# LeSN-Lab/diff-ViT

Hardware: AMD Instinct MI355X
Metric: images/sec DeiT-S int8 224^2 b=256 (quantized forward) (higher is better)
Workload: dtype int8; 1 GPU; deit_small PoT-PTQ forward, bit_config=[8]*50, 224x224, batch 256 per GPU; global_batch=256, parallelism=dp1, streams_per_gpu=3, collective=none, ranks_seen=1, distinct_devices=1

## Files before the change

### diff-vit_amd/csrc/p2vit_capi.cpp

```cpp
#include <hip/hip_runtime.h>
#include <math.h>
#include <stdarg.h>
#include <stdio.h>
#include <stdlib.h>
#include <string.h>

#include <initializer_list>
#include <memory>
#include <vector>

#include "p2vit_kernels.h"

static thread_local char g_err[512] = "";

static int fail(int code, const char* fmt, ...) {
  va_list ap;
  va_start(ap, fmt);
  vsnprintf(g_err, sizeof g_err, fmt, ap);
  va_end(ap);
  return code;
}
static bool stream_capturing(void* stream) {
  hipStreamCaptureStatus status = hipStreamCaptureStatusNone;
  if (hipStreamIsCapturing((hipStream_t)stream, &status) != hipSuccess) {
    (void)hipGetLastError();
    return false;
  }
  return status == hipStreamCaptureStatusActive;
}
static int refuse_capture(const char* who, const char* why, void* stream) {
  if (!stream_capturing(stream)) return P2V_OK;
  return fail(P2V_E_UNSUPPORTED, "%s: the stream is capturing a HIP graph and this call %s; make it outside the capture", who, why);
}
struct KeepLastError {
  char keep[sizeof g_err];
  KeepLastError() { memcpy(keep, g_err, sizeof keep); }
  ~KeepLastError() { memcpy(g_err, keep, sizeof keep); }
};
static int launch_rc(int rc, const char* what) {
  if (rc == 0) return 0;
  if (rc == -2) return fail(P2V_E_UNSUPPORTED, "%s: s_qkv_sq * inv_s_attn must be a power of two", what);
  if (rc < 0) return fail(P2V_E_UNSUPPORTED, "%s: no kernel instantiated for this shape", what);
  return fail(P2V_E_LAUNCH, "%s: %s", what, hipGetErrorString((hipError_t)rc));
}
static inline int round_up(int v, int m) { return (v + m - 1) / m * m; }
static bool is_pot(float v) {
  int ex;
  return v > 0.f && frexpf(v, &ex) == 0.5f;
}

static int check_lis_consts(const char* who, int x0_int, int b_int, int c_int) {
  if (x0_int >= 0) return fail(P2V_E_ARG, "%s: x0_int must be negative", who);
  if (c_int <= 0 || c_int >= (1 << 24) || b_int < 0 || b_int >= (1 << 23) || x0_int < -(1 << 12))
    return fail(P2V_E_UNSUPPORTED, "%s: log-int-softmax constants out of range (x0 %d, b %d, c %d): softmax input scale below 2^-11?", who, x0_int,
                b_int, c_int);
  return P2V_OK;
}
static int check_requant_scale(const char* who, float inv_s_out) {
  if (!(is_pot(inv_s_out) && inv_s_out >= 0x1p-40f && inv_s_out <= 0x1p40f))
    return fail(P2V_E_UNSUPPORTED, "%s: REQUANT 1/scale %g must be a power of two (it is folded into the column scales)", who, inv_s_out);
  return P2V_OK;
}
static int check_gelu_tab(const char* who, const p2v_gelu_tab& t) {
  if (t.table && (t.cells <= 0 || t.cells > 4096)) return fail(P2V_E_ARG, "%s: GELU table with %d cells", who, t.cells);
  return P2V_OK;
}
static int check_softmax_bits(const char* who, int bits) {
  if (bits != 3 && bits != 4) return fail(P2V_E_UNSUPPORTED, "%s: softmax_bits %d (the log-int-softmax runs at 3 or 4 bits)", who, bits);
  return P2V_OK;
}
static float av_mul_max(int bits) { return bits == 3 ? 0x1p7f : 0x1p15f; }
static int check_attn(const char* who, const p2v_attn& at, int bits = 4) {
  if (const int rb = check_softmax_bits(who, bits)) return rb;
  const int rc = check_lis_consts(who, at.x0_int, at.b_int, at.c_int);
  if (rc != P2V_OK) return rc;
  if (!is_pot(at.s_qkv_sq * at.inv_s_attn)) return fail(P2V_E_UNSUPPORTED, "%s: s_qkv_sq * inv_s_attn must be a power of two", who);
  if (!(at.qk_scale > 0.f) || !(at.av_mul > 0.f)) return fail(P2V_E_ARG, "%s: qk_scale and av_mul must be positive", who);
  if (!is_pot(at.av_mul) || at.av_mul > av_mul_max(bits) || at.av_mul < 0x1p-40f)
    return fail(P2V_E_UNSUPPORTED, "%s: av_mul %g must be a power of two in [2^-40, 2^%d] at softmax_bits %d", who, at.av_mul, bits == 3 ? 7 : 15, bits);
  return P2V_OK;
}

struct p2v_plan {
  p2v_model_desc d;
  int tokens, patches, k_patch, k_patch_pad, n_layers;
  std::vector<p2v_linear> lin[2];
  std::vector<char> lin_set[2];
  float inv_s_input;
  p2v_epilogue embed_epi;
  const int8_t* cls_codes;
  const int8_t* embed_cls_codes = nullptr;
  bool embed_set;
  std::vector<p2v_block> blocks;
  std::vector<char> block_set;
  p2v_ln final_ln;
  float head_inv_s, head_s;
  bool head_set;
  std::vector<float*> ln_pre_buf;
  float* final_pre_buf = nullptr;
  std::vector<char> block_folded;
  std::vector<const float*> resid_tab;
  std::vector<float*> resid_buf;
  int device = -1;
  bool float_norm = false, float_softmax = false, fhead_set = false;
  std::vector<p2v_float_block> fblocks;
  std::vector<char> fblock_set;
  p2v_float_ln final_fln = {};
  std::vector<char> softmax_bits;
  struct GramScale { const float* scale; const uint8_t* shift; double unit; };
  std::vector<GramScale> gram_scales;
  uint8_t* gram_shift_buf = nullptr;
  bool grams_ready = false;
  ~p2v_plan() {
    int prev = -1;
    const bool sw = device >= 0 && hipGetDevice(&prev) == hipSuccess && prev != device && hipSetDevice(device) == hipSuccess;
    for (float* b : ln_pre_buf)
      if (b) (void)hipFree(b);
    for (float* b : resid_buf)
      if (b) (void)hipFree(b);
    if (final_pre_buf) (void)hipFree(final_pre_buf);
    if (gram_shift_buf) (void)hipFree(gram_shift_buf);
    if (sw) (void)hipSetDevice(prev);
  }
};

static void build_resid_tables(p2v_plan* plan, int block);
static int bit_index(int bits) { return bits == 4 ? 0 : (bits == 8 ? 1 : -1); }
template <class Block>
static auto& block_ln(Block& b, int i) { return i < 2 ? b.ln1[i] : b.ln2[(i - 2) >> 1][(i - 2) & 1]; }
static bool ln_constants_present(const p2v_ln& l, bool with_mask = true) {
  return (l.mask || !with_mask) && l.gamma && l.beta && l.inv_out && l.post_mul;
}

extern "C" {

extern int g_ln_generic;
extern int g_ln_rows;
extern int g_attn_waves;
extern int g_ln_gemm;
extern int g_ln_gemm_ver;
extern int g_gemm_tile;
extern int g_resid_pre;
extern int g_attn_stream;
extern int g_attn_packed;
extern int g_ln_pre;
extern int g_gemm_rows;
int g_cls_rows = 1;

enum { ANY_ENV = 1, ANY_API = 2 };
static const struct Switch {
  const char *name, *env;
  int* var;
  int lo, hi, step, any;
  bool takes(int v, int how) const { return (any & how) || (v >= lo && v <= hi && (v - lo) % step == 0); }
  void set(int v) const { *var = (hi == 1 && lo == 0) ? v != 0 : v; }
} kSwitches[] = {
    {"attn_waves", "P2V_ATTN_WAVES", &g_attn_waves, 4, 8, 1, 0},
    {"ln_gemm", "P2V_LN_GEMM", &g_ln_gemm, 0, 1, 1, ANY_ENV | ANY_API},
    {"ln_gemm_version", "P2V_LN_GEMM_V", &g_ln_gemm_ver, 1, 3, 1, 0},
    {"gemm_tile", "P2V_GEMM_TILE", &g_gemm_tile, 0, 256, 128, 0},
    {"attn_stream", "P2V_ATTN_STREAM", &g_attn_stream, 0, 1, 1, ANY_ENV | ANY_API},
    {"attn_packed", "P2V_ATTN_PACKED", &g_attn_packed, 0, 1, 1, 0},
    {"ln_pre", "P2V_LN_PRE", &g_ln_pre, 0, 1, 1, ANY_ENV | ANY_API},
    {"resid_pre", "P2V_RESID_PRE", &g_resid_pre, 0, 1, 1, ANY_ENV | ANY_API},
    {"gemm_rows", "P2V_GEMM_ROWS", &g_gemm_rows, 0, 2, 1, 0},
    {"cls_rows", "P2V_CLS_ROWS", &g_cls_rows, 0, 1, 1, ANY_ENV},
    {"ln_rows", "P2V_LN_ROWS", &g_ln_rows, 1, 64, 1, 0},
    {"ln_generic", "P2V_LN_GENERIC", &g_ln_generic, 0, 1, 1, ANY_API},
};

static void read_env_once() {
  static bool done = false;
  if (done) return;
  done = true;
  for (const Switch& s : kSwitches) {
    const char* e = getenv(s.env);
    if (e && s.takes(atoi(e), ANY_ENV)) s.set(atoi(e));
  }
}
int p2v_abi_version(void) { read_env_once(); return P2V_ABI_VERSION; }

int p2v_resident_tokens(int head_dim) { return p2v_resident_tokens_of(head_dim); }
int p2v_max_tokens(int head_dim) { return p2v_resident_tokens_of(head_dim) ? P2V_MAX_TOKENS_STREAMED : 0; }
int p2v_packed_tokens(int head_dim) { return head_dim == 64 ? P2V_MAX_TOKENS_PACKED : 0; }
int p2v_attention_kernel(int head_dim, int tokens, int tapped) {
  read_env_once();
  return p2v_attention_kernel_of(head_dim, tokens, tapped);
}

int p2v_set_tuning(const char* name, int value) {
  if (!name) return fail(P2V_E_ARG, "p2v_set_tuning: null name");
  read_env_once();
  for (const Switch& s : kSwitches)
    if (!strcmp(name, s.name) && s.takes(value, ANY_API)) {
      s.set(value);
      return P2V_OK;
    }
  return fail(P2V_E_ARG, "p2v_set_tuning: unknown switch or value out of range: %s = %d", name, value);
}
const char* p2v_last_error(void) { return g_err; }

int p2v_plan_create(const p2v_model_desc* desc, p2v_plan** out) {
  if (!desc || !out) return fail(P2V_E_ARG, "p2v_plan_create: null argument");
  read_env_once();
  if (desc->abi_version != P2V_ABI_VERSION) return fail(P2V_E_ARG, "ABI version %d != %d", desc->abi_version, P2V_ABI_VERSION);
  const p2v_model_desc& d = *desc;
  if (d.img_size <= 0 || d.patch_size <= 0 || d.img_size % d.patch_size) return fail(P2V_E_SHAPE, "img_size %% patch_size != 0");
  if (d.patch_size % 4) return fail(P2V_E_UNSUPPORTED, "patch_size must be a multiple of 4");
  if (d.embed_dim % d.num_heads) return fail(P2V_E_SHAPE, "embed_dim %% num_heads != 0");
  const int hd = d.embed_dim / d.num_heads;
  if (hd != 32 && hd != 48 && hd != 64 && hd != 80 && hd != 96 && hd != 128)
    return fail(P2V_E_UNSUPPORTED, "head_dim %d (32, 48, 64, 80, 96 and 128 are instantiated)", hd);
  if (d.embed_dim % 16 || d.mlp_hidden % 16) return fail(P2V_E_UNSUPPORTED, "embed_dim and mlp_hidden must be multiples of 16");
  {
    const int tokens = (d.img_size / d.patch_size) * (d.img_size / d.patch_size) + 1;
    if (tokens > P2V_MAX_TOKENS_STREAMED)
      return fail(P2V_E_UNSUPPORTED, "%d tokens per image: the attention kernels cover up to %d", tokens, P2V_MAX_TOKENS_STREAMED);
  }
  if (d.embed_dim > 2048) return fail(P2V_E_UNSUPPORTED, "embed_dim %d: the LayerNorm kernel covers up to 2048 channels", d.embed_dim);
  p2v_plan* p = new p2v_plan();
  p->d = d;
  p->patches = (d.img_size / d.patch_size) * (d.img_size / d.patch_size);
  p->tokens = p->patches + 1;
  p->k_patch = d.in_chans * d.patch_size * d.patch_size;
  p->k_patch_pad = round_up(p->k_patch, GBK_PAD);
  p->n_layers = 4 * d.depth + 2;
  for (int b = 0; b < 2; ++b) {
    p->lin[b].assign(p->n_layers, p2v_linear{nullptr, nullptr, nullptr, nullptr, 0});
    p->lin_set[b].assign(p->n_layers, 0);
  }
  p->blocks.resize(d.depth);
  p->block_set.assign(d.depth, 0);
  p->ln_pre_buf.assign(d.depth, nullptr);
  p->block_folded.assign(d.depth, 0);
  p->resid_tab.assign((size_t)d.depth * 4, nullptr);
  p->resid_buf.assign(d.depth, nullptr);
  p->embed_set = p->head_set = false;
  p->cls_codes = nullptr;
  p->fblocks.resize(d.depth);
  p->fblock_set.assign(d.depth, 0);
  p->softmax_bits.assign(d.depth, 4);
  *out = p;
  return P2V_OK;
}

void p2v_plan_destroy(p2v_plan* plan) { delete plan; }

int p2v_plan_set_linear(p2v_plan* plan, int layer, int bits, const p2v_linear* lin) {
  if (!plan || !lin) return fail(P2V_E_ARG, "p2v_plan_set_linear: null argument");
  const int bi = bit_index(bits);
  if (bi < 0) return fail(P2V_E_BITS, "bits %d not in {4, 8}", bits);
  if (layer < 0 || layer >= plan->n_layers) return fail(P2V_E_ARG, "layer %d out of range [0,%d)", layer, plan->n_layers);
  if (!lin->w_codes || !lin->colscale || !lin->bias) return fail(P2V_E_ARG, "p2v_plan_set_linear: null device pointer");
  if (lin->packed4 && bits != 4) return fail(P2V_E_BITS, "packed4 weights for a %d-bit layer", bits);
  plan->lin[bi][layer] = *lin;
  plan->lin_set[bi][layer] = 1;
  if (layer >= 1 && layer < plan->n_layers - 1 && ((layer - 1) & 1)) {
    const int block = (layer - 1) / 4;
    if (plan->block_set[block]) build_resid_tables(plan, block);
  }
  return P2V_OK;
}

int p2v_plan_set_embed(p2v_plan* plan, float inv_s_input, const p2v_epilogue* e, const int8_t* cls_row_codes) {
  if (!plan || !e || !cls_row_codes) return fail(P2V_E_ARG, "p2v_plan_set_embed: null argument");
  plan->inv_s_input = inv_s_input;
  plan->embed_epi = *e;
  plan->embed_epi.patches = plan->patches;
  plan->cls_codes = cls_row_codes;
  plan->embed_set = true;
  return P2V_OK;
}

int p2v_plan_set_embed_tap_cls(p2v_plan* plan, const int8_t* cls_embed_codes) {
  if (!plan || !cls_embed_codes) return fail(P2V_E_ARG, "p2v_plan_set_embed_tap_cls: null argument");
  plan->embed_cls_codes = cls_embed_codes;
  return P2V_OK;
}

struct OwnerDevice {
  int prev = -1, own = -1;
  explicit OwnerDevice(const void* ptr) {
    hipPointerAttribute_t pa;
    if (hipGetDevice(&prev) != hipSuccess || hipPointerGetAttributes(&pa, ptr) != hipSuccess) {
      (void)hipGetLastError();
      return;
    }
    if (pa.type != hipMemoryTypeDevice && pa.type != hipMemoryTypeManaged) return;
    own = pa.device;
    if (own != prev && hipSetDevice(own) != hipSuccess) own = -1;
  }
  ~OwnerDevice() { if (own >= 0 && own != prev) (void)hipSetDevice(prev); }
  bool ok() const { return own >= 0; }
};

static size_t resid_tab_floats(int N) { return (size_t)((N + 127) / 128) * 6 * 128; }

static int resid_prefold_impl(const p2v_linear& lin, const p2v_epilogue& ep, int N, float* tab, int* usable, hipStream_t st) {
  *usable = 0;
  unsigned* flags = nullptr;
  hipError_t e = hipMalloc(&flags, 2 * sizeof(unsigned));
  const unsigned init[2] = {1u, 0u};
  unsigned got[2] = {0u, 0u};
  if (e == hipSuccess) e = hipMemcpyAsync(flags, init, sizeof init, hipMemcpyHostToDevice, st);
  int rc = 0;
  if (e == hipSuccess) rc = p2v_launch_resid_prefold(lin, ep, N, tab, flags, st);
  if (e == hipSuccess && rc == 0) e = hipMemcpyAsync(got, flags, sizeof got, hipMemcpyDeviceToHost, st);
  if (e == hipSuccess && rc == 0) e = hipStreamSynchronize(st);
  if (flags) (void)hipFree(flags);
  if (e != hipSuccess) {
    (void)hipGetLastError();
    return fail(P2V_E_LAUNCH, "resid_prefold: %s", hipGetErrorString(e));
  }
  if (rc) return launch_rc(rc, "resid_prefold");
  *usable = got[0] ? 1 : 0;
  return P2V_OK;
}

static void build_resid_tables(p2v_plan* plan, int block) {
  KeepLastError keep;
  for (int j = 0; j < 4; ++j) plan->resid_tab[(size_t)block * 4 + j] = nullptr;
  if (!plan->block_set[block]) return;
  const p2v_block& blk = plan->blocks[block];
  OwnerDevice dev(blk.proj_epi.s_mid);
  if (!dev.ok() || (plan->device >= 0 && plan->device != dev.own)) return;
  const int D = plan->d.embed_dim;
  const size_t per = resid_tab_floats(D);
  if (hipDeviceSynchronize() != hipSuccess) { (void)hipGetLastError(); return; }
  float* buf = plan->resid_buf[block];
  if (!buf && hipMalloc(&buf, 4 * per * sizeof(float)) != hipSuccess) { (void)hipGetLastError(); return; }
  plan->resid_buf[block] = buf;
  plan->device = dev.own;
  for (int which = 0; which < 2; ++which)
    for (int bi = 0; bi < 2; ++bi) {
      const int layer = 1 + 4 * block + (which ? 3 : 1);
      if (!plan->lin_set[bi][layer]) continue;
      int usable = 0;
      float* tab = buf + (size_t)(which * 2 + bi) * per;
      if (resid_prefold_impl(plan->lin[bi][layer], which ? blk.fc2_epi : blk.proj_epi, D, tab, &usable, nullptr) == P2V_OK && usable)
        plan->resid_tab[(size_t)block * 4 + which * 2 + bi] = tab;
    }
}

static hipError_t fold_one_ln(const p2v_ln& l, int C, float* dev, p2v_ln_pre* out) {
  const int Cp = round_up(C, 256);
  std::vector<float> g(C), b(C), io(C), pm(C), host((size_t)2 * Cp, 0.f);
  hipError_t e = hipMemcpy(g.data(), l.gamma, C * sizeof(float), hipMemcpyDeviceToHost);
  if (e == hipSuccess) e = hipMemcpy(b.data(), l.beta, C * sizeof(float), hipMemcpyDeviceToHost);
  if (e == hipSuccess) e = hipMemcpy(io.data(), l.inv_out, C * sizeof(float), hipMemcpyDeviceToHost);
  if (e == hipSuccess) e = hipMemcpy(pm.data(), l.post_mul, C * sizeof(float), hipMemcpyDeviceToHost);
  if (e != hipSuccess) return e;
  float* go = host.data();
  float* bo = go + Cp;
  int pot = 1, pm1 = 1;
  float gmin = 3.0e38f, gmax = 0.f, bmax = 0.f;
  for (int c = 0; c < C; ++c) {
    unsigned ib;
    memcpy(&ib, &io[c], 4);
    const int p2 = (int)((ib & 0x807FFFFFu) == 0u) & (int)((ib >> 23) - 32u <= 190u);
    go[c] = g[c] * io[c];
    bo[c] = b[c] * io[c];
    const float ga = fabsf(go[c]), ba = fabsf(bo[c]);
    const int gok = (int)(g[c] == 0.f) | ((int)(ga >= 1.0e-30f) & (int)(ga <= 1.0e30f));
    const int bok = (int)(b[c] == 0.f) | ((int)(ba >= 1.0e-30f) & (int)(ba <= 1.0e30f));
    pot &= p2 & gok & bok;
    pm1 &= (int)(pm[c] == 1.f);
    gmin = fminf(gmin, ga);
    gmax = fmaxf(gmax, ga);
    bmax = fmaxf(bmax, ba);
  }
  e = hipMemcpy(dev, host.data(), host.size() * sizeof(float), hipMemcpyHostToDevice);
  if (e == hipSuccess) *out = p2v_ln_pre{dev, dev + Cp, gmin, gmax, bmax, pot, pm1};
  return e;
}
static const p2v_ln_pre kNoPre = {nullptr, nullptr, 0.f, 0.f, 0.f, 0, 0};

static bool fold_ln_constants(p2v_plan* plan, int block) {
  const int C = plan->d.embed_dim, Cp = round_up(C, 256);
  p2v_block& blk = plan->blocks[block];
  for (int i = 0; i < 6; ++i) block_ln(blk, i).pre = kNoPre;
  OwnerDevice own(blk.ln1[0].gamma);
  if (!own.ok()) {
    fail(P2V_OK, "p2v_plan_set_block: LayerNorm constants of block %d not folded at plan time (cannot locate the device of gamma)", block);
    return false;
  }
  if (plan->device >= 0 && plan->device != own.own) {
    fail(P2V_OK, "p2v_plan_set_block: block %d lives on device %d, earlier blocks on device %d: not folded at plan time", block, own.own, plan->device);
    return false;
  }
  hipError_t e = hipDeviceSynchronize();
  float* dev = plan->ln_pre_buf[block];
  if (e == hipSuccess && !dev) e = hipMalloc(&dev, (size_t)12 * Cp * sizeof(float));
  p2v_ln_pre pre[6];
  if (e == hipSuccess) {
    plan->ln_pre_buf[block] = dev;
    plan->device = own.own;
    for (int i = 0; i < 6 && e == hipSuccess; ++i) e = fold_one_ln(block_ln(blk, i), C, dev + (size_t)(2 * i) * Cp, &pre[i]);
  }
  if (e != hipSuccess) {
    (void)hipGetLastError();
    fail(P2V_OK, "p2v_plan_set_block: LayerNorm constants of block %d not folded at plan time (%s)", block, hipGetErrorString(e));
    return false;
  }
  for (int i = 0; i < 6; ++i) block_ln(blk, i).pre = pre[i];
  return true;
}

int p2v_plan_set_block(p2v_plan* plan, int block, const p2v_block* blk) {
  if (!plan || !blk) return fail(P2V_E_ARG, "p2v_plan_set_block: null argument");
  if (block < 0 || block >= plan->d.depth) return fail(P2V_E_ARG, "block %d out of range", block);
  int rc = check_attn("p2v_plan_set_block: attn", blk->attn, plan->softmax_bits[block]);
  if (rc == P2V_OK) rc = check_gelu_tab("p2v_plan_set_block: gelu_fc1", blk->gelu_fc1);
  for (int b = 0; b < 2 && rc == P2V_OK; ++b) rc = check_requant_scale("p2v_plan_set_block: inv_s_qkv", blk->inv_s_qkv[b]);
  if (rc == P2V_OK && !(is_pot(blk->inv_s_fc1) && blk->inv_s_fc1 >= 0x1p-40f && blk->inv_s_fc1 <= 0x1p40f))
    rc = fail(P2V_E_UNSUPPORTED, "p2v_plan_set_block: 1/scale of mlp.qact1 %g must be a power of two", blk->inv_s_fc1);
  if (rc == P2V_OK && (!blk->proj_epi.s_mid || !blk->proj_epi.s_res || !blk->proj_epi.s_next || !blk->fc2_epi.s_mid || !blk->fc2_epi.s_res ||
                       !blk->fc2_epi.s_next))
    rc = fail(P2V_E_ARG, "p2v_plan_set_block: RESID epilogues need s_mid/s_res/s_next");
  for (int i = 0; i < 6 && rc == P2V_OK; ++i)
    if (!ln_constants_present(block_ln(*blk, i))) rc = fail(P2V_E_ARG, "p2v_plan_set_block: LayerNorm constants missing");
  if (rc != P2V_OK) return rc;
  plan->blocks[block] = *blk;
  plan->block_set[block] = 1;
  g_err[0] = 0;
  plan->block_folded[block] = fold_ln_constants(plan, block) ? 1 : 0;
  build_resid_tables(plan, block);
  return P2V_OK;
}

int p2v_plan_block_prefolded(const p2v_plan* plan, int block) {
  if (!plan || block < 0 || block >= plan->d.depth) return fail(P2V_E_ARG, "p2v_plan_block_prefolded: bad argument");
  return plan->block_folded[block] ? 1 : 0;
}

int p2v_plan_resid_prefolded(const p2v_plan* plan, int block) {
  if (!plan || block < 0 || block >= plan->d.depth) return fail(P2V_E_ARG, "p2v_plan_resid_prefolded: bad argument");
  int m = 0;
  for (int j = 0; j < 4; ++j) m |= plan->resid_tab[(size_t)block * 4 + j] ? 1 << j : 0;
  return m;
}

int p2v_plan_set_head(p2v_plan* plan, const p2v_ln* final_ln, float inv_s_out, float s_out) {
  if (!plan || !final_ln) return fail(P2V_E_ARG, "p2v_plan_set_head: null argument");
  if (!ln_constants_present(*final_ln))
    return fail(P2V_E_ARG, "p2v_plan_set_head: LayerNorm constants missing");
  if (!(inv_s_out > 0.f) || !(s_out > 0.f)) return fail(P2V_E_ARG, "p2v_plan_set_head: act_out scale must be positive");
  plan->final_ln = *final_ln;
  plan->final_ln.pre = kNoPre;
  {
    OwnerDevice own(final_ln->gamma);
    const int C = plan->d.embed_dim;
    if (own.ok() && (plan->device < 0 || plan->device == own.own) && hipDeviceSynchronize() == hipSuccess) {
      if (!plan->final_pre_buf && hipMalloc(&plan->final_pre_buf, (size_t)2 * round_up(C, 256) * sizeof(float)) != hipSuccess) plan->final_pre_buf = nullptr;
      p2v_ln_pre pre;
      if (plan->final_pre_buf && fold_one_ln(*final_ln, C, plan->final_pre_buf, &pre) == hipSuccess) {
        plan->final_ln.pre = pre;
        plan->device = own.own;
      }
    }
    (void)hipGetLastError();
  }
  plan->head_inv_s = inv_s_out;
  plan->head_s = s_out;
  plan->head_set = true;
  return P2V_OK;
}

struct WsLayout {
  size_t patches, x, ln, qkv, att, hid, cls, total;
};
static WsLayout ws_layout(const p2v_plan* p, int batch) {
// ... 1807 lines not shown
```

### diff-vit_amd/csrc/p2vit_ln.hip

```cpp
#include "p2vit_ln_row.h"
#include "p2vit_launch.h"


#ifndef LN_BATCH
#define LN_BATCH 2
#endif
#ifndef LN_LDSC
#define LN_LDSC true
#endif
template <int NCH, int LANES, bool PRE, bool TAP = false>
__global__ __launch_bounds__(256) void k_int_layernorm(LnArgs a) {
  __shared__ __attribute__((aligned(16))) float sG[NCH * LANES * 4], sB[NCH * LANES * 4], sP[NCH * LANES * 4];
  __shared__ __attribute__((aligned(16))) int sM[NCH * LANES * 4];
  const int tid = threadIdx.x, l32 = tid & (LANES - 1), hw = tid / LANES;
  LnLane<NCH, LN_LDSC> L;
  const int LN_ROWS = a.rows_per_half;
  const long long row0 = ((long long)blockIdx.x * (256 / LANES) + hw) * LN_ROWS;
  const long long last_row = a.rows - 1;
  constexpr int R = LN_BATCH;
  int colofs[NCH];
#pragma unroll
  for (int i = 0; i < NCH; ++i) colofs[i] = (l32 + LANES * i) * 4 < a.C ? (l32 + LANES * i) * 4 : 0;
  unsigned wnext[R][NCH];
#pragma unroll
  for (int u = 0; u < R; ++u)
#pragma unroll
    for (int i = 0; i < NCH; ++i)
      wnext[u][i] = *reinterpret_cast<const unsigned*>(a.x + (row0 + u < a.rows ? row0 + u : last_row) * a.row_stride + colofs[i]);
  if constexpr (PRE) {
#pragma unroll
    for (int i = 0; i < NCH; ++i) {
      const int c = (l32 + LANES * i) * 4;
      L.on[i] = c < a.C;
      L.gm[i] = *reinterpret_cast<const float4*>(a.pre.gm + c);
      L.bt[i] = *reinterpret_cast<const float4*>(a.pre.bt + c);
    }
    for (int t4 = tid; t4 < NCH * LANES; t4 += 256) {
      const int c = t4 * 4;
      float4 pmv = make_float4(0.f, 0.f, 0.f, 0.f), mk = pmv;
      if (c < a.C) {
        pmv = *reinterpret_cast<const float4*>(a.ln.post_mul + c);
        mk = *reinterpret_cast<const float4*>(a.ln.mask + c);
      }
      *reinterpret_cast<float4*>(sP + c) = pmv;
      *reinterpret_cast<float4*>(sM + c) = ln_scale_mask(mk);
    }
    __syncthreads();
#pragma unroll
    for (int i = 0; i < NCH; ++i) {
      const int c = (l32 + LANES * i) * 4;
      if constexpr (sizeof(L.pm) == sizeof(float4) * NCH) {
        L.pm[i] = *reinterpret_cast<const float4*>(sP + c);
        L.mkf[i] = *reinterpret_cast<const float4*>(sM + c);
      }
    }
    L.sPl = sP + l32 * 4;
    L.sMl = reinterpret_cast<const float*>(sM) + l32 * 4;
    L.cstride = LANES * 4;
    L.gmin = a.pre.gmin;
    L.gmax = a.pre.gmax;
    L.bmax = a.pre.bmax;
    L.pot = a.pre.pot != 0 && a.force_generic == 0;
    L.pm_one = a.pre.pm_one != 0;
  } else {
    ln_prepare<NCH, LANES>(a.ln, a.C, a.force_generic != 0, sG, sB, sP, sM, tid, 256, L);
  }
#pragma unroll
  for (int u = 0; u < R; ++u)
#pragma unroll
    for (int i = 0; i < NCH; ++i) asm volatile("" : "+v"(wnext[u][i]));
#pragma unroll 1
  for (int rr = 0; rr < LN_ROWS; rr += R) {
    const long long row = row0 + rr;
    if (row >= a.rows) break;
    unsigned wcur[R][NCH];
#pragma unroll
    for (int u = 0; u < R; ++u)
#pragma unroll
      for (int i = 0; i < NCH; ++i) wcur[u][i] = L.on[i] ? wnext[u][i] : 0u;
#pragma unroll
    for (int u = 0; u < R; ++u) {
      const long long nrow = row + R + u < a.rows ? row + R + u : last_row;
#pragma unroll
      for (int i = 0; i < NCH; ++i) wnext[u][i] = *reinterpret_cast<const unsigned*>(a.x + nrow * a.row_stride + colofs[i]);
    }
    asm volatile("" ::: "memory");
    unsigned outw[R][NCH];
    if constexpr (TAP) {
      float* taps[R];
#pragma unroll
      for (int u = 0; u < R; ++u) taps[u] = (rr + u < LN_ROWS && row + u < a.rows) ? a.tap_out + (row + u) * (long long)a.C : nullptr;
      if constexpr (R == 1) ln_row<NCH, LANES, decltype(L), true>(wcur[0], L, a.ln, a.C, l32, outw[0], taps[0]);
      else ln_rows<NCH, LANES, R, decltype(L), true>(wcur, L, a.ln, a.C, l32, outw, taps);
    } else {
    if constexpr (R == 1) ln_row<NCH, LANES>(wcur[0], L, a.ln, a.C, l32, outw[0]);
    else ln_rows<NCH, LANES, R>(wcur, L, a.ln, a.C, l32, outw);
    }
#pragma unroll
    for (int u = 0; u < R; ++u)
#pragma unroll
      for (int i = 0; i < NCH; ++i) asm volatile("" : "+v"(wnext[u][i]));
#pragma unroll
    for (int u = 0; u < R; ++u) {
      if (rr + u >= LN_ROWS || row + u >= a.rows) continue;
      int8_t* dst = a.out + (row + u) * a.out_stride;
#pragma unroll
      for (int i = 0; i < NCH; ++i)
        if (L.on[i]) *reinterpret_cast<unsigned*>(dst + (l32 + LANES * i) * 4) = outw[u][i];
    }
  }
}

#define LG_BM 64
template <bool W4> struct LgW { typedef uint4 raw; };
template <> struct LgW<true> { typedef uint2 raw; };
__device__ __forceinline__ v4i lg_wfrag(uint4 w) { return __builtin_bit_cast(v4i, w); }
__device__ __forceinline__ v4i lg_wfrag(uint2 w) { return unpack_w4(w.x, w.y); }
struct LnGemmLds {
  int panel, consts, fold, table, total;
};
__host__ __device__ inline LnGemmLds ln_gemm_lds(int K, int N, int nch, int table_cells) {
  LnGemmLds o;
  const int kt = (K + GBK - 1) / GBK, tiles_n = (N + GBN - 1) / GBN;
  o.panel = 0;
  o.consts = o.panel + kt * LG_BM * GBK;
  o.fold = o.panel;
  o.table = o.consts + tiles_n * GBN * 2 * (int)sizeof(float);
  o.total = o.table + table_cells * 8;
  return o;
}

#ifdef P2V_DIAG
#define LG_STAMP(slot)                                                                                              \
  do {                                                                                                              \
    if (g.stamps && threadIdx.x == 0 && (slot) < 62) g.stamps[(long long)blockIdx.x * 64 + (slot)] = __builtin_readcyclecounter(); \
  } while (0)
#else
#define LG_STAMP(slot) do { } while (0)
#endif
template <int EPI, int KT, bool W4>
__global__ __launch_bounds__(256, 2) void k_ln_gemm(LnArgs a, GemmArgs g) {
  typedef typename LgW<W4>::raw wraw;
  constexpr int NCH = (KT + 1) / 2;
  constexpr int NI = 2 * KT;
  extern __shared__ __attribute__((aligned(1024))) unsigned char lg_smem[];
  LG_STAMP(0);
  const int C = a.C;
  const int cells = EPI == P2V_EPI_GELU_TAB ? g.ep.gelu.cells : 0;
  const LnGemmLds lay = ln_gemm_lds(C, g.N, NCH, cells);
  int8_t* panel = reinterpret_cast<int8_t*>(lg_smem + lay.panel);
  float* consts = reinterpret_cast<float*>(lg_smem + lay.consts);
  const unsigned char* gtab = lg_smem + lay.table;
  const int tid = threadIdx.x, lane = tid & 63;
  const int wave = __builtin_amdgcn_readfirstlane(tid >> 6);
  const int h = lane >> 5, l31 = lane & 31;
  const int m0 = blockIdx.x * LG_BM;
  const int tiles_n = g.tiles_n;

  const wraw* wsrc = reinterpret_cast<const wraw*>(g.W) + (long long)wave * NI * 64 + lane;
  wraw wf[NI];
#pragma unroll
  for (int i = 0; i < NI; ++i) wf[i] = wsrc[i * 64];

  constexpr int RPH = LG_BM / 8;
  static_assert(RPH % 2 == 0, "rows are processed in pairs");
  const int hw = tid >> 5;
  auto load_row = [&](int r, unsigned (&w)[NCH]) {
    long long row = (long long)m0 + hw * RPH + r;
    row = row < a.rows ? row : a.rows - 1;
#pragma unroll
    for (int i = 0; i < NCH; ++i) {
      const int c = (l31 + 32 * i) * 4;
      w[i] = *reinterpret_cast<const unsigned*>(a.x + row * a.row_stride + (c < C ? c : 0));
    }
  };
  unsigned win[2][NCH];
  load_row(0, win[0]);
  load_row(1, win[1]);
  {
    const float fold = EPI == P2V_EPI_REQUANT ? g.ep.inv_s_out : (EPI == P2V_EPI_GELU_TAB ? g.ep.gelu.k : 1.0f);
    const float cfold = fold * (W4 ? 0.0625f : 1.0f);
    for (int n4 = tid; n4 < tiles_n * (GBN / 4); n4 += 256) {
      const int j_ = n4 >> 5, c_ = (n4 & 31) * 4;
      const float4 cv = *reinterpret_cast<const float4*>(g.colscale + n4 * 4);
      const float4 bv = *reinterpret_cast<const float4*>(g.bias + n4 * 4);
      *reinterpret_cast<float4*>(consts + j_ * 2 * GBN + c_) = make_float4(cv.x * cfold, cv.y * cfold, cv.z * cfold, cv.w * cfold);
      *reinterpret_cast<float4*>(consts + j_ * 2 * GBN + GBN + c_) = make_float4(bv.x * fold, bv.y * fold, bv.z * fold, bv.w * fold);
    }
    if (EPI == P2V_EPI_GELU_TAB)
      for (int i = tid; i < cells; i += 256)
        reinterpret_cast<uint2*>(lg_smem + lay.table)[i] = reinterpret_cast<const uint2*>(g.ep.gelu.table)[i];
  }
  LG_STAMP(1);
  {
    float* sG = reinterpret_cast<float*>(lg_smem + lay.fold);
    float* sB = sG + NCH * 128;
    float* sP = sB + NCH * 128;
    int* sM = reinterpret_cast<int*>(sP + NCH * 128);
    LnLane<NCH> L;
    ln_prepare<NCH, 32>(a.ln, C, a.force_generic != 0, sG, sB, sP, sM, tid, 256, L);
    __syncthreads();
#pragma unroll 1
    for (int r = 0; r < RPH; r += 2) {
      unsigned wnext[2][NCH];
      if (r + 2 < RPH) {
        load_row(r + 2, wnext[0]);
        load_row(r + 3, wnext[1]);
      }
      unsigned wcur[2][NCH], outw2[2][NCH];
#pragma unroll
      for (int u = 0; u < 2; ++u)
#pragma unroll
        for (int i = 0; i < NCH; ++i) wcur[u][i] = L.on[i] ? win[u][i] : 0u;
      ln_rows<NCH, 32, 2>(wcur, L, a.ln, C, l31, outw2);
#pragma unroll
      for (int u = 0; u < 2; ++u) {
        const int lrow = hw * RPH + r + u;
        const unsigned (&outw)[NCH] = outw2[u];
        const long long row = (long long)m0 + lrow;
#pragma unroll
        for (int i = 0; i < NCH; ++i) {
          const int c = (l31 + 32 * i) * 4;
          if (c < KT * GBK)
            *reinterpret_cast<unsigned*>(panel + (c >> 6) * (LG_BM * GBK) + lrow * GBK + ((((c & 63) >> 4) ^ ((lrow >> 2) & 3)) << 4) + (c & 15)) =
                L.on[i] ? outw[i] : 0u;
          if (a.out && L.on[i] && row < a.rows) *reinterpret_cast<unsigned*>(a.out + row * a.out_stride + c) = outw[i];
        }
      }
      if (r + 2 < RPH) {
#pragma unroll
        for (int i = 0; i < NCH; ++i) {
          win[0][i] = wnext[0][i];
          win[1][i] = wnext[1][i];
        }
      }
    }
  }
  LG_STAMP(2);
  __syncthreads();
  LG_STAMP(3);

  const int8_t* pXa = panel + lds_off64(l31, h);
  const int8_t* pXb = panel + lds_off64(32 + l31, h);
  const int xks = (lds_off64(l31, 2 + h) - lds_off64(l31, h));
  v16i acc[2];
#pragma unroll
  for (int b = 0; b < 2; ++b)
#pragma unroll
    for (int r = 0; r < 16; ++r) acc[b][r] = 0;

  for (int j = 0; j < tiles_n; ++j) {
    const bool more = j + 1 < tiles_n;
    const wraw* wnext = wsrc + (long long)(more ? j + 1 : j) * 4 * NI * 64;
#pragma unroll
    for (int i = 0; i < NI; ++i) {
      const int off = (i >> 1) * (LG_BM * GBK) + (i & 1) * xks;
      const v4i xa = *reinterpret_cast<const v4i*>(pXa + off);
      const v4i xb = *reinterpret_cast<const v4i*>(pXb + off);
      const v4i wfi = lg_wfrag(wf[i]);
      acc[0] = __builtin_amdgcn_mfma_i32_32x32x32_i8(wfi, xa, acc[0], 0, 0, 0);
      acc[1] = __builtin_amdgcn_mfma_i32_32x32x32_i8(wfi, xb, acc[1], 0, 0, 0);
      wf[i] = wnext[i * 64];
    }
    LG_STAMP(4 + 2 * j);
    const EpiLds* e = reinterpret_cast<const EpiLds*>(consts + j * 2 * GBN);
    {
      const uint4 nores[2] = {make_uint4(0, 0, 0, 0), make_uint4(0, 0, 0, 0)};
      gemm_epilogue_tile2<EPI>(acc, m0 + l31, j * GBN + 32 * wave, 32 * wave, h, g, e, nores, gtab);
#pragma unroll
      for (int mi = 0; mi < 2; ++mi)
#pragma unroll
        for (int r = 0; r < 16; ++r) acc[mi][r] = 0;
    }
    LG_STAMP(5 + 2 * j);
  }
}

template <int NI>
__host__ __device__ constexpr int lg2_mfma_at(int hp) {
  for (int q = 0; q < 2 * NI; ++q)
    if ((q * 12) / NI == hp) return q;
  return -1;
}

#ifndef LG2_LN_ROWS
#define LG2_LN_ROWS 2
#endif
template <int EPI, int KT, int NG, bool W4>
__global__ __launch_bounds__(256 * NG, 2) void k_ln_gemm2(LnArgs a, GemmArgs g) {
  typedef typename LgW<W4>::raw wraw;
  constexpr int NT = 256 * NG;
  static_assert(EPI == P2V_EPI_REQUANT || EPI == P2V_EPI_GELU_TAB, "pipelined epilogues");
  constexpr int NCH = (KT + 1) / 2;
  constexpr int NI = 2 * KT;
  extern __shared__ __attribute__((aligned(1024))) unsigned char lg_smem[];
  LG_STAMP(0);
  const int C = a.C;
  const int cells = EPI == P2V_EPI_GELU_TAB ? g.ep.gelu.cells : 0;
  const LnGemmLds lay = ln_gemm_lds(C, g.N, NCH, cells);
  int8_t* panel = reinterpret_cast<int8_t*>(lg_smem + lay.panel);
  float* consts = reinterpret_cast<float*>(lg_smem + lay.consts);
  const unsigned char* gtab = lg_smem + lay.table;
  const int tid = threadIdx.x, lane = tid & 63;
  const int wave = __builtin_amdgcn_readfirstlane(tid >> 6);
  const int grp = NG == 1 ? 0 : (wave >> 2), cw = wave & 3;
  const int h = lane >> 5, l31 = lane & 31;
  const int m0 = blockIdx.x * LG_BM;
  const int tiles_n = g.tiles_n;
  const int n_g = (tiles_n - grp + NG - 1) / NG;

  const wraw* wsrc = reinterpret_cast<const wraw*>(g.W) + (long long)cw * NI * 64 + lane;
  auto wtile = [&](int it) {
    int j = grp + NG * it;
    j = j < tiles_n ? j : tiles_n - 1;
    return wsrc + (long long)j * 4 * NI * 64;
  };
  constexpr int NI_EARLY = KT >= 6 ? NI - 1 : NI;
  wraw wf[NI];
  {
    const wraw* w0 = wtile(0);
#pragma unroll
    for (int i = 0; i < NI_EARLY; ++i) wf[i] = w0[i * 64];
  }

  constexpr int RPH = LG_BM / (8 * NG);
  static_assert(RPH % 2 == 0, "rows are processed in pairs");
  const int hw = tid >> 5;
  const int8_t* xblk = a.x + (long long)m0 * a.row_stride;
  const int rstride = (int)a.row_stride;
  const int last_lr = (int)(a.rows - 1 - m0);
  auto load_row = [&](int r, unsigned (&w)[NCH]) {
    int lr = hw * RPH + r;
    lr = lr < last_lr ? lr : last_lr;
    const int8_t* rp = xblk + lr * rstride;
#pragma unroll
    for (int i = 0; i < NCH; ++i) {
      const int c = (l31 + 32 * i) * 4;
      w[i] = *reinterpret_cast<const unsigned*>(rp + (c < C ? c : 0));
    }
  };
  constexpr int LR = LG2_LN_ROWS < RPH ? LG2_LN_ROWS : RPH;
  static_assert(RPH % LR == 0, "rows are processed in batches");
  unsigned win[LR][NCH];
#pragma unroll
  for (int u = 0; u < LR; ++u) load_row(u, win[u]);
  {
    const float fold = EPI == P2V_EPI_REQUANT ? g.ep.inv_s_out : (EPI == P2V_EPI_GELU_TAB ? g.ep.gelu.k : 1.0f);
    const float cfold = fold * (W4 ? 0.0625f : 1.0f);
    for (int n4 = tid; n4 < tiles_n * (GBN / 4); n4 += NT) {
      const int j_ = n4 >> 5, c_ = (n4 & 31) * 4;
      const float4 cv = *reinterpret_cast<const float4*>(g.colscale + n4 * 4);
      const float4 bv = *reinterpret_cast<const float4*>(g.bias + n4 * 4);
      *reinterpret_cast<float4*>(consts + j_ * 2 * GBN + c_) = make_float4(cv.x * cfold, cv.y * cfold, cv.z * cfold, cv.w * cfold);
      *reinterpret_cast<float4*>(consts + j_ * 2 * GBN + GBN + c_) = make_float4(bv.x * fold, bv.y * fold, bv.z * fold, bv.w * fold);
    }
    if (EPI == P2V_EPI_GELU_TAB)
      for (int i = tid; i < cells; i += NT)
        reinterpret_cast<uint2*>(lg_smem + lay.table)[i] = reinterpret_cast<const uint2*>(g.ep.gelu.table)[i];
  }
  LG_STAMP(1);
  {
    float* sG = reinterpret_cast<float*>(lg_smem + lay.fold);
    float* sB = sG + NCH * 128;
    float* sP = sB + NCH * 128;
    int* sM = reinterpret_cast<int*>(sP + NCH * 128);
    LnLane<NCH> L;
    if (a.pre.gm) {
#pragma unroll
      for (int i = 0; i < NCH; ++i) {
        const int c = (l31 + 32 * i) * 4;
        L.on[i] = c < C;
        L.gm[i] = *reinterpret_cast<const float4*>(a.pre.gm + c);
        L.bt[i] = *reinterpret_cast<const float4*>(a.pre.bt + c);
        L.pm[i] = L.on[i] ? *reinterpret_cast<const float4*>(a.ln.post_mul + c) : make_float4(0.f, 0.f, 0.f, 0.f);
        L.mkf[i] = L.on[i] ? ln_scale_mask(*reinterpret_cast<const float4*>(a.ln.mask + c)) : make_float4(0.f, 0.f, 0.f, 0.f);
      }
      L.gmin = a.pre.gmin;
      L.gmax = a.pre.gmax;
      L.bmax = a.pre.bmax;
      L.pot = a.pre.pot != 0 && a.force_generic == 0;
      L.pm_one = a.pre.pm_one != 0;
    } else {
      ln_prepare<NCH, 32>(a.ln, C, a.force_generic != 0, sG, sB, sP, sM, tid, NT, L);
      __syncthreads();
    }
#pragma unroll 1
    for (int r = 0; r < RPH; r += LR) {
      unsigned wnext[LR][NCH];
      if (r + LR < RPH) {
#pragma unroll
        for (int u = 0; u < LR; ++u) load_row(r + LR + u, wnext[u]);
      }
      unsigned wcur[LR][NCH], outw2[LR][NCH];
#pragma unroll
      for (int u = 0; u < LR; ++u)
#pragma unroll
        for (int i = 0; i < NCH; ++i) wcur[u][i] = L.on[i] ? win[u][i] : 0u;
      ln_rows<NCH, 32, LR>(wcur, L, a.ln, C, l31, outw2);
#pragma unroll
      for (int u = 0; u < LR; ++u) {
        const int lrow = hw * RPH + r + u;
        const unsigned (&outw)[NCH] = outw2[u];
        const long long row = (long long)m0 + lrow;
#pragma unroll
        for (int i = 0; i < NCH; ++i) {
          const int c = (l31 + 32 * i) * 4;
          if (c < KT * GBK)
            *reinterpret_cast<unsigned*>(panel + (c >> 6) * (LG_BM * GBK) + lrow * GBK + ((((c & 63) >> 4) ^ ((lrow >> 2) & 3)) << 4) + (c & 15)) =
                L.on[i] ? outw[i] : 0u;
          if (a.out && L.on[i] && row < a.rows) *reinterpret_cast<unsigned*>(a.out + row * a.out_stride + c) = outw[i];
        }
      }
      if (r + LR < RPH) {
#pragma unroll
        for (int u = 0; u < LR; ++u)
#pragma unroll
          for (int i = 0; i < NCH; ++i) win[u][i] = wnext[u][i];
      }
    }
  }
  LG_STAMP(2);
  if constexpr (NI_EARLY < NI) wf[NI - 1] = wtile(0)[(NI - 1) * 64];
  __syncthreads();
  LG_STAMP(3);
  if (n_g <= 0) return;

  const int8_t* pXa = panel + lds_off64(l31, h);
  const int8_t* pXb = panel + lds_off64(32 + l31, h);
  const int xks = (lds_off64(l31, 2 + h) - lds_off64(l31, h));
#define LG2_XOFF(i) ((((i) >> 1) * (LG_BM * GBK)) + (((i) & 1) ? xks : 0))
  v16i acc[2], accn[2];
#pragma unroll
  for (int b = 0; b < 2; ++b)
#pragma unroll
    for (int r = 0; r < 16; ++r) acc[b][r] = 0;
  {
    const wraw* wn = wtile(1);
#pragma unroll
    for (int i = 0; i < NI; ++i) {
      const v4i xa = *reinterpret_cast<const v4i*>(pXa + LG2_XOFF(i));
      const v4i xb = *reinterpret_cast<const v4i*>(pXb + LG2_XOFF(i));
      const v4i wfi = lg_wfrag(wf[i]);
      acc[0] = __builtin_amdgcn_mfma_i32_32x32x32_i8(wfi, xa, acc[0], 0, 0, 0);
      acc[1] = __builtin_amdgcn_mfma_i32_32x32x32_i8(wfi, xb, acc[1], 0, 0, 0);
      wf[i] = wn[i * 64];
    }
  }
  LG_STAMP(4);
  v4i XA[2], XB[2];
  XA[0] = *reinterpret_cast<const v4i*>(pXa + LG2_XOFF(0));
  XB[0] = *reinterpret_cast<const v4i*>(pXb + LG2_XOFF(0));
  XA[1] = XA[0];
  XB[1] = XB[0];
  const int goff = (int)g.ep.gelu.off;
  const float glo = (float)-goff, ghi = (float)(cells - 1 - goff) + 0.5f;
  const unsigned char* gtabz = gtab + goff * 8;

  v4i wcur = {0, 0, 0, 0};
  auto tile_body = [&](auto MFc, auto LDc, auto COPYc, int j, const wraw* wnn, v16i (&acc)[2], v16i (&accn)[2]) {
    constexpr bool MF = decltype(MFc)::value, LD = decltype(LDc)::value, COPY = decltype(COPYc)::value;
    const float* cst = consts + j * 2 * GBN + 32 * cw + 4 * h;
    const int n_tile = j * GBN + 32 * cw;
    unsigned d[2][4];
    float4 cs = *reinterpret_cast<const float4*>(cst), bs = *reinterpret_cast<const float4*>(cst + GBN);
#define LG2_MFMA(HP)                                                                                                     \
    do {                                                                                                                 \
      constexpr int q_ = lg2_mfma_at<NI>(HP);                                                                            \
      if constexpr (MF && q_ >= 0) {                                                                                     \
        constexpr int i_ = q_ >> 1, nx_ = (i_ + 1) % NI;                                                                 \
        if constexpr ((q_ & 1) == 0) {                                                                                   \
          XA[nx_ & 1] = *reinterpret_cast<const v4i*>(pXa + LG2_XOFF(nx_));                                              \
          wcur = lg_wfrag(wf[i_]);                                                                                       \
          if constexpr (i_ == 0) accn[0] = __builtin_amdgcn_mfma_i32_32x32x32_i8(wcur, XA[i_ & 1], (v16i){0,0,0,0,0,0,0,0,0,0,0,0,0,0,0,0}, 0, 0, 0); \
          else accn[0] = __builtin_amdgcn_mfma_i32_32x32x32_i8(wcur, XA[i_ & 1], accn[0], 0, 0, 0);                      \
        } else {                                                                                                         \
          XB[nx_ & 1] = *reinterpret_cast<const v4i*>(pXb + LG2_XOFF(nx_));                                              \
          if constexpr (i_ == 0) accn[1] = __builtin_amdgcn_mfma_i32_32x32x32_i8(wcur, XB[i_ & 1], (v16i){0,0,0,0,0,0,0,0,0,0,0,0,0,0,0,0}, 0, 0, 0); \
          else accn[1] = __builtin_amdgcn_mfma_i32_32x32x32_i8(wcur, XB[i_ & 1], accn[1], 0, 0, 0);                      \
          if constexpr (LD) wf[i_] = wnn[i_ * 64];                                                                       \
        }                                                                                                                \
      }                                                                                                                  \
    } while (0)
#define LG2_FENCE() __builtin_amdgcn_sched_barrier(0)
    auto group = [&](auto GQc) {
      constexpr int gq = decltype(GQc)::value;
      const float4 csc = cs, bsc = bs;
      if (gq < 3) {
        cs = *reinterpret_cast<const float4*>(cst + 8 * (gq + 1));
        bs = *reinterpret_cast<const float4*>(cst + GBN + 8 * (gq + 1));
      }
      float y0[4], y1[4];
      LG2_MFMA(6 * gq + 0);
      y0[0] = __builtin_fmaf((float)acc[0][4 * gq + 0], csc.x, bsc.x);
      y0[1] = __builtin_fmaf((float)acc[0][4 * gq + 1], csc.y, bsc.y);
      y0[2] = __builtin_fmaf((float)acc[0][4 * gq + 2], csc.z, bsc.z);
      y0[3] = __builtin_fmaf((float)acc[0][4 * gq + 3], csc.w, bsc.w);
      LG2_FENCE();
      LG2_MFMA(6 * gq + 1);
      y1[0] = __builtin_fmaf((float)acc[1][4 * gq + 0], csc.x, bsc.x);
      y1[1] = __builtin_fmaf((float)acc[1][4 * gq + 1], csc.y, bsc.y);
      y1[2] = __builtin_fmaf((float)acc[1][4 * gq + 2], csc.z, bsc.z);
      y1[3] = __builtin_fmaf((float)acc[1][4 * gq + 3], csc.w, bsc.w);
      LG2_FENCE();
      if constexpr (EPI == P2V_EPI_GELU_TAB) {
        uint2 e0[4], e1[4];
        LG2_MFMA(6 * gq + 2);
#pragma unroll
        for (int i = 0; i < 4; ++i) e0[i] = *reinterpret_cast<const uint2*>(gtabz + gelu_tab_offset(y0[i], glo, ghi));
        LG2_FENCE();
        LG2_MFMA(6 * gq + 3);
#pragma unroll
        for (int i = 0; i < 4; ++i) e1[i] = *reinterpret_cast<const uint2*>(gtabz + gelu_tab_offset(y1[i], glo, ghi));
        LG2_FENCE();
        LG2_MFMA(6 * gq + 4);
        d[0][gq] = 0;
        P2V_GELU_SEL(0, "UNUSED_PAD", d[0][gq], y0[0], e0[0]);
        P2V_GELU_SEL(1, "UNUSED_PRESERVE", d[0][gq], y0[1], e0[1]);
        P2V_GELU_SEL(2, "UNUSED_PRESERVE", d[0][gq], y0[2], e0[2]);
        P2V_GELU_SEL(3, "UNUSED_PRESERVE", d[0][gq], y0[3], e0[3]);
        LG2_FENCE();
        LG2_MFMA(6 * gq + 5);
        d[1][gq] = 0;
        P2V_GELU_SEL(0, "UNUSED_PAD", d[1][gq], y1[0], e1[0]);
        P2V_GELU_SEL(1, "UNUSED_PRESERVE", d[1][gq], y1[1], e1[1]);
        P2V_GELU_SEL(2, "UNUSED_PRESERVE", d[1][gq], y1[2], e1[2]);
        P2V_GELU_SEL(3, "UNUSED_PRESERVE", d[1][gq], y1[3], e1[3]);
        LG2_FENCE();
      } else {
        float r0[4], r1[4];
        LG2_MFMA(6 * gq + 2);
#pragma unroll
        for (int i = 0; i < 4; ++i) r0[i] = pre_pack(y0[i]);
        LG2_FENCE();
        LG2_MFMA(6 * gq + 3);
#pragma unroll
        for (int i = 0; i < 4; ++i) r1[i] = pre_pack(y1[i]);
        LG2_FENCE();
        LG2_MFMA(6 * gq + 4);
        d[0][gq] = pack4_pre(r0[0], r0[1], r0[2], r0[3]);
        LG2_FENCE();
        LG2_MFMA(6 * gq + 5);
        d[1][gq] = pack4_pre(r1[0], r1[1], r1[2], r1[3]);
        LG2_FENCE();
      }
    };
    group(std::integral_constant<int, 0>{});
    group(std::integral_constant<int, 1>{});
    group(std::integral_constant<int, 2>{});
    group(std::integral_constant<int, 3>{});
#undef LG2_MFMA
#undef LG2_FENCE
#pragma unroll
    for (int b = 0; b < 2; ++b) {
      const uint4 o = halves_to_row16(d[b][0], d[b][1], d[b][2], d[b][3]);
      const int m = m0 + 32 * b + l31;
      if (m < g.M && n_tile + 16 * h < g.N)
        *reinterpret_cast<uint4*>(reinterpret_cast<int8_t*>(g.out) + (long long)m * g.ldo + n_tile + 16 * h) = o;
    }
    if constexpr (MF && COPY) {
      acc[0] = accn[0];
      acc[1] = accn[1];
    }
  };
  using T_ = std::integral_constant<bool, true>;
  using F_ = std::integral_constant<bool, false>;
  int it = 0;
  for (; it + 3 < n_g; it += 2) {
    tile_body(T_{}, T_{}, F_{}, grp + NG * it, wtile(it + 2), acc, accn);
    LG_STAMP(5 + it);
    tile_body(T_{}, T_{}, F_{}, grp + NG * (it + 1), wtile(it + 3), accn, acc);
    LG_STAMP(6 + it);
  }
  if (it + 2 < n_g) {
    tile_body(T_{}, T_{}, T_{}, grp + NG * it, wtile(it + 2), acc, accn);
    LG_STAMP(5 + it);
    ++it;
  }
  if (it + 1 < n_g) {
    tile_body(T_{}, F_{}, T_{}, grp + NG * it, wsrc, acc, accn);
    LG_STAMP(5 + it);
    ++it;
  }
  tile_body(F_{}, F_{}, T_{}, grp + NG * it, wsrc, acc, accn);
  LG_STAMP(5 + it);
#undef LG2_XOFF
}


#ifdef P2V_DIAG
extern unsigned long long* g_gemm_stamps;
#endif
int g_ln_pre = 1;
int g_ln_generic = 0;
int g_ln_gemm = 1;
bool p2v_ln_gemm_supported(int epi, int C, int N, int table_cells) {
  if (!g_ln_gemm || (epi != P2V_EPI_REQUANT && epi != P2V_EPI_GELU)) return false;
  if (C % 4 || C > 384 || N % 16) return false;
  return ln_gemm_lds(C, N, ((C + GBK - 1) / GBK + 1) / 2, table_cells).total <= 80 * 1024;
}
template <int EPI, int KT, int VER, bool W4>
static int launch_ln_gemm_t(const LnArgs& a, const GemmArgs& g, int cells, hipStream_t st) {
  constexpr auto kernel = [] {
    if constexpr (VER == 1) return &k_ln_gemm<EPI, KT, W4>;
    else return &k_ln_gemm2<EPI, KT, VER - 1, W4>;
  }();
  const int smem = ln_gemm_lds(a.C, g.N, (KT + 1) / 2, cells).total;
  static P2vLdsGrant grant = {};
  const hipError_t e = grant.ensure(reinterpret_cast<const void*>(kernel), smem);
  if (e != hipSuccess) return (int)e;
  const dim3 grid((unsigned)((g.M + LG_BM - 1) / LG_BM));
  hipLaunchKernelGGL(kernel, grid, dim3(VER == 3 ? 512 : 256), (unsigned)smem, st, a, g);
  CHECK_LAUNCH();
  return 0;
}
typedef int (*LnGemmLauncher)(const LnArgs&, const GemmArgs&, int, hipStream_t);
constexpr int kLnGemmEpi[3] = {P2V_EPI_REQUANT, P2V_EPI_GELU_TAB, P2V_EPI_GELU};
constexpr int ln_gemm_index(int e, int ver, int kt, bool w4) { return (((3 - ver) * 3 + p2v_slot(kLnGemmEpi, e)) * 6 + kt - 1) * 2 + (w4 ? 0 : 1); }
struct LnGemmAt {
  template <int I> static constexpr LnGemmLauncher at() {
    constexpr int E = kLnGemmEpi[I / 12 % 3], VER = 3 - I / 36;
    static_assert(ln_gemm_index(E, VER, I / 2 % 6 + 1, !(I & 1)) == I, "decoded as the launcher encodes");
    if constexpr (E != P2V_EPI_GELU || VER == 1) return launch_ln_gemm_t<E, I / 2 % 6 + 1, VER, !(I & 1)>;
    else return nullptr;
  }
};
static const auto ln_gemm_table = p2v_table<LnGemmLauncher, LnGemmAt, 108>();

int g_ln_gemm_ver = 2;
int p2v_launch_ln_gemm(int epi, const LnArgs& a_, const GemmArgs& g0, hipStream_t st) {
  const int cells = (epi == P2V_EPI_GELU && g0.ep.gelu.table) ? g0.ep.gelu.cells : 0;
  if (!p2v_ln_gemm_supported(epi, a_.C, g0.N, cells)) return -3;
  if (a_.row_stride < 0 || a_.row_stride > (1 << 24)) return -3;
  LnArgs a = a_;
  a.force_generic = g_ln_generic;
  if (!g_ln_pre) a.pre.gm = nullptr;
  GemmArgs g = g0;
  g.tiles_n = (g.N + GBN - 1) / GBN;
#ifdef P2V_DIAG
  g.stamps = g_gemm_stamps;
#endif
  const int kt = (a.C + GBK - 1) / GBK;
  const int e = epi == P2V_EPI_REQUANT ? P2V_EPI_REQUANT : (cells ? P2V_EPI_GELU_TAB : P2V_EPI_GELU);
  const int ver = ((g_ln_gemm_ver == 3 || g_ln_gemm_ver == 2) && !g.ep.tap_out && e != P2V_EPI_GELU) ? g_ln_gemm_ver : 1;
  const LnGemmLauncher launch = ln_gemm_table[ln_gemm_index(e, ver, kt >= 1 && kt <= 5 ? kt : 6, g.w4 != 0)];
  return launch ? launch(a, g, cells, st) : -3;
}

typedef void (*LnKernel)(LnArgs);
constexpr int ln_index(bool tap, bool half, int nch, bool pre) { return (((tap ? 0 : 2) + (half ? 1 : 0)) * 9 + nch) * 2 + (pre ? 0 : 1); }
struct LnAt {
  template <int I> static constexpr LnKernel at() {
    constexpr bool HALF = (I / 18 & 1) != 0;
    constexpr int NCH = I / 2 % 9;
    static_assert(ln_index(I < 36, HALF, NCH, !(I & 1)) == I, "decoded as the launcher encodes");
    if constexpr (HALF ? (NCH >= 1 && NCH <= 3) : (NCH >= 2 && NCH <= 8)) return k_int_layernorm<NCH, HALF ? 32 : 64, !(I & 1), (I < 36)>;
    else return nullptr;
  }
};
static const auto ln_table = p2v_table<LnKernel, LnAt, 72>();

int g_ln_rows = 4;
int p2v_launch_layernorm(const LnArgs& a_, hipStream_t st) {
  LnArgs a = a_;
  a.force_generic = g_ln_generic;
  if (!g_ln_pre) a.pre.gm = nullptr;
  if (a.C > 2048) return a.tap_out ? -1 : p2v_launch_layernorm_xwide(a, st);
  a.rows_per_half = g_ln_rows;
  const int LN_ROWS = g_ln_rows;
  const bool wide = a.C > 384;
  const int nch = wide ? (a.C + 255) / 256 : (a.C + 127) / 128;
  const int rows_per_block = (wide ? 4 : 8) * LN_ROWS;
  dim3 grid((unsigned)((a.rows + rows_per_block - 1) / rows_per_block)), block(256);
  const LnKernel kernel = (nch >= 0 && nch <= 8) ? ln_table[ln_index(a.tap_out != nullptr, !wide, nch, a.pre.gm != nullptr)] : nullptr;
  if (!kernel) return -1;
  hipLaunchKernelGGL(kernel, grid, block, 0, st, a);
  CHECK_LAUNCH();
  return 0;
}
```

### diff-vit_amd/csrc/p2vit_ln_row.h

```cpp
#pragma once
#include "p2vit_epilogue.h"

__device__ __forceinline__ int half_wave_sum(int v) {
  v += __builtin_amdgcn_update_dpp(0, v, 0xB1, 0xF, 0xF, false);
  v += __builtin_amdgcn_update_dpp(0, v, 0x4E, 0xF, 0xF, false);
  v += __builtin_amdgcn_update_dpp(0, v, 0x141, 0xF, 0xF, false);
  v += __builtin_amdgcn_update_dpp(0, v, 0x140, 0xF, 0xF, false);
  v += __builtin_amdgcn_ds_swizzle(v, 0x401F);
  return v;
}

__device__ __forceinline__ float ln_elem_generic_o(float xq, float g, float bta, float io, float rs, float mos, float os) {
  const float A = os > 0.f ? (rs * g) / os : (rs * g) * io;
  const float absA = fabsf(A);
  int N = 134 - (int)(__float_as_uint(absA) >> 23);
  N = N < 0 ? 0 : (N > 31 ? 31 : N);
  const float M = fminf(floorf(ldexpf(absA, N)), 255.f);
  const float sM = copysignf(M, A);
  const float tb = bta - mos * g;
  const float Bv = rintf(ldexpf(os > 0.f ? tb / os : tb * io, N));
  return rintf(ldexpf(sM * xq + Bv, -N));
}
__device__ __forceinline__ float ln_elem_generic(float xq, float g, float bta, float io, float pm, float rs, float mos, float os) {
  const float o = ln_elem_generic_o(xq, g, bta, io, rs, mos, os);
  return rintf(o * pm);
}

#define LN_XS 0x1p-16f
#define LN_XS_INV 65536.f
__device__ __forceinline__ float4 ln_scale_mask(float4 m) { return make_float4(m.x * LN_XS, m.y * LN_XS, m.z * LN_XS, m.w * LN_XS); }
template <int NCH, bool LDSC = false>
struct LnLane {
  bool on[NCH];
  float4 gm[NCH], bt[NCH];
  float4 pm[LDSC ? 1 : NCH];
  float4 mkf[LDSC ? 1 : NCH];
  const float* sPl;
  const float* sMl;
  int cstride;
  float gmin, gmax;
  float bmax;
  bool pot;
  bool pm_one;
  __device__ __forceinline__ float4 post4(int i) const { return LDSC ? *reinterpret_cast<const float4*>(sPl + i * cstride) : pm[LDSC ? 0 : i]; }
  __device__ __forceinline__ float4 mask4(int i) const { return LDSC ? *reinterpret_cast<const float4*>(sMl + i * cstride) : mkf[LDSC ? 0 : i]; }
};

template <int NCH, int LANES, class LL>
__device__ __forceinline__ void ln_prepare(const p2v_ln& ln, int C, bool force_generic, float* sG, float* sB, float* sP, int* sM,
                                           int tid, int nthreads, LL& L) {
  const int l32 = tid & (LANES - 1);
  int potf = force_generic ? 0 : 1, pm1 = 1;
  for (int t4 = tid; t4 < NCH * LANES; t4 += nthreads) {
    const int c = t4 * 4;
    float4 g = make_float4(0.f, 0.f, 0.f, 0.f), b = g, io = make_float4(1.f, 1.f, 1.f, 1.f), pmv = g, mk = g;
    if (c < C) {
      g = *reinterpret_cast<const float4*>(ln.gamma + c);
      b = *reinterpret_cast<const float4*>(ln.beta + c);
      io = *reinterpret_cast<const float4*>(ln.inv_out + c);
      pmv = *reinterpret_cast<const float4*>(ln.post_mul + c);
      mk = *reinterpret_cast<const float4*>(ln.mask + c);
    }
    const float g4[4] = {g.x, g.y, g.z, g.w}, b4[4] = {b.x, b.y, b.z, b.w}, i4[4] = {io.x, io.y, io.z, io.w};
    if (c < C) pm1 &= (int)(pmv.x == 1.f) & (int)(pmv.y == 1.f) & (int)(pmv.z == 1.f) & (int)(pmv.w == 1.f);
    float go[4], bo[4];
#pragma unroll
    for (int j = 0; j < 4; ++j) {
      const unsigned ib = __float_as_uint(i4[j]);
      const int p2 = (int)((ib & 0x807FFFFFu) == 0u) & (int)((ib >> 23) - 32u <= 190u);
      go[j] = g4[j] * i4[j];
      bo[j] = b4[j] * i4[j];
      const float ga = fabsf(go[j]), ba = fabsf(bo[j]);
      const int gok = (int)(g4[j] == 0.f) | ((int)(ga >= 1.0e-30f) & (int)(ga <= 1.0e30f));
      const int bok = (int)(b4[j] == 0.f) | ((int)(ba >= 1.0e-30f) & (int)(ba <= 1.0e30f));
      potf &= p2 & gok & bok;
    }
    *reinterpret_cast<float4*>(sG + c) = make_float4(go[0], go[1], go[2], go[3]);
    *reinterpret_cast<float4*>(sB + c) = make_float4(bo[0], bo[1], bo[2], bo[3]);
    *reinterpret_cast<float4*>(sP + c) = pmv;
    *reinterpret_cast<float4*>(sM + c) = ln_scale_mask(mk);
  }
  L.pot = __syncthreads_and(potf) != 0;
  L.pm_one = __syncthreads_and(pm1) != 0;
  float gmin = 3.0e38f, gmax = 0.f, bmax = 0.f;
#pragma unroll
  for (int i = 0; i < NCH; ++i) {
    const int c = (l32 + LANES * i) * 4;
    L.on[i] = c < C;
    const float4 gv = *reinterpret_cast<const float4*>(sG + c);
    L.gm[i] = gv;
    L.bt[i] = *reinterpret_cast<const float4*>(sB + c);
    if (L.on[i]) bmax = fmaxf(bmax, fmaxf(fmaxf(fabsf(L.bt[i].x), fabsf(L.bt[i].y)), fmaxf(fabsf(L.bt[i].z), fabsf(L.bt[i].w))));
    if constexpr (sizeof(L.pm) == sizeof(float4) * NCH) {
      L.pm[i] = *reinterpret_cast<const float4*>(sP + c);
      L.mkf[i] = *reinterpret_cast<const float4*>(sM + c);
    }
    const float lo = fminf(fminf(fabsf(gv.x), fabsf(gv.y)), fminf(fabsf(gv.z), fabsf(gv.w)));
    const float hi = fmaxf(fmaxf(fabsf(gv.x), fabsf(gv.y)), fmaxf(fabsf(gv.z), fabsf(gv.w)));
    gmin = fminf(gmin, L.on[i] ? lo : 3.0e38f);
    gmax = fmaxf(gmax, L.on[i] ? hi : 0.f);
  }
  L.sPl = sP + l32 * 4;
  L.sMl = reinterpret_cast<const float*>(sM) + l32 * 4;
  L.cstride = LANES * 4;
  {
    int lo = (int)__float_as_uint(gmin), hi = (int)__float_as_uint(gmax), bh = (int)__float_as_uint(bmax);
#define LN_MM(ctrl) lo = min(lo, __builtin_amdgcn_update_dpp(lo, lo, ctrl, 0xF, 0xF, false)); hi = max(hi, __builtin_amdgcn_update_dpp(hi, hi, ctrl, 0xF, 0xF, false)); \
                    bh = max(bh, __builtin_amdgcn_update_dpp(bh, bh, ctrl, 0xF, 0xF, false));
    LN_MM(0xB1) LN_MM(0x4E) LN_MM(0x141) LN_MM(0x140)
#undef LN_MM
    lo = min(lo, __builtin_amdgcn_ds_swizzle(lo, 0x401F));
    hi = max(hi, __builtin_amdgcn_ds_swizzle(hi, 0x401F));
    bh = max(bh, __builtin_amdgcn_ds_swizzle(bh, 0x401F));
    if (LANES >= 64) {
      lo = min(lo, __shfl_xor(lo, 32));
      hi = max(hi, __shfl_xor(hi, 32));
      bh = max(bh, __shfl_xor(bh, 32));
    }
    L.gmin = __uint_as_float((unsigned)lo);
    L.gmax = __uint_as_float((unsigned)hi);
    L.bmax = __uint_as_float((unsigned)bh);
  }
}

template <int NCH, class LL>
__device__ __forceinline__ void ln_sums(const unsigned (&wcur)[NCH], const LL& L, float (&xq)[NCH][4], int& S1, unsigned& S2) {
  S2 = 0;
  float S1p = 0.f, S2p = 0.f;
#pragma unroll
  for (int i = 0; i < NCH; ++i) {
    const unsigned w = wcur[i];
    const float4 mk_ = L.mask4(i);
    const float m4[4] = {mk_.x, mk_.y, mk_.z, mk_.w};
#pragma unroll
    for (int j = 0; j < 4; ++j) xq[i][j] = (float)sx8(w, j) * m4[j];
    S1p += (xq[i][0] + xq[i][1]) + (xq[i][2] + xq[i][3]);
    S2p += __builtin_fmaf(xq[i][1], xq[i][1], xq[i][0] * xq[i][0]) + __builtin_fmaf(xq[i][3], xq[i][3], xq[i][2] * xq[i][2]);
    if ((i & 3) == 3 || i == NCH - 1) {
      S2 += (unsigned)(S2p * (LN_XS_INV * LN_XS_INV));
      S2p = 0.f;
    }
  }
  S1 = (int)(S1p * LN_XS_INV);
}
template <int LANES>
__device__ __forceinline__ void ln_reduce(int& S1, unsigned& S2) {
  S1 = half_wave_sum(S1);
  S2 = (unsigned)half_wave_sum((int)S2);
  if (LANES == 64) {
    S1 += __shfl_xor(S1, 32);
    S2 += (unsigned)__shfl_xor((int)S2, 32);
  }
}
template <int NCH, class LL>
__device__ __forceinline__ void ln_scalars(int S1, unsigned S2, const LL& L, const p2v_ln& ln, int C, float& rs, float& mos, bool& fast) {
  const float s1 = ln.s1;
  const float Cf = (float)C;
  const float s1oC = s1 / Cf;
  const float S1f = (float)S1, S2f = (float)S2;
  const float mean = (S1f / Cf) * s1;
  const float stdv = s1oC * sqrtf(Cf * S2f - S1f * S1f);
  rs = s1 / stdv;
  mos = mean / stdv;
  const float amin = rs * L.gmin;
  const float tlim = __uint_as_float((((__float_as_uint(amin) >> 23) & 255u) + 15u) << 23);
  fast = L.pot && amin >= 0x1p-24f && rs * L.gmax < 256.f && (L.bmax + fabsf(mos) * L.gmax) * 1.01f < tlim;
}
__device__ __forceinline__ void ln_tap_store(float* tap, int c, const p2v_ln& ln, const float (&o)[4]) {
  float4 os;
  if (ln.out_scale) {
    os = *reinterpret_cast<const float4*>(ln.out_scale + c);
  } else {
    const float4 io = *reinterpret_cast<const float4*>(ln.inv_out + c);
    os = make_float4(1.0f / io.x, 1.0f / io.y, 1.0f / io.z, 1.0f / io.w);
  }
  *reinterpret_cast<float4*>(tap + c) = make_float4(o[0] * os.x, o[1] * os.y, o[2] * os.z, o[3] * os.w);
}

template <int NCH, int LANES, class LL, bool TAP = false>
__device__ __forceinline__ void ln_apply(const float (&xq)[NCH][4], const LL& L, const p2v_ln& ln, int l32, float rs, float mos, bool fast,
                                         unsigned (&outw)[NCH], float* tap = nullptr) {
  if (fast) {
    const float rs2 = rs * LN_XS_INV;
    auto chain = [&](auto PM1c) {
      constexpr bool PM1 = decltype(PM1c)::value;
#pragma unroll
      for (int i = 0; i < NCH; ++i) {
        const float g4[4] = {L.gm[i].x, L.gm[i].y, L.gm[i].z, L.gm[i].w}, b4[4] = {L.bt[i].x, L.bt[i].y, L.bt[i].z, L.bt[i].w};
        float p4[4] = {1.f, 1.f, 1.f, 1.f};
        if constexpr (!PM1) {
          const float4 pm_ = L.post4(i);
          p4[0] = pm_.x; p4[1] = pm_.y; p4[2] = pm_.z; p4[3] = pm_.w;
        }
        float q[4];
        float ot[TAP ? 4 : 1];
#pragma unroll
        for (int j = 0; j < 4; j += 2) {
          v2f T2, Bq2;
#pragma unroll
          for (int e = 0; e < 2; ++e) {
            const float A2 = rs2 * g4[j + e];
            const float t = b4[j + e] - mos * g4[j + e];
            const unsigned Ab = __float_as_uint(A2);
            T2[e] = __uint_as_float(Ab & 0xFFFF0000u);
            unsigned Cmb;
            asm("v_and_or_b32 %0, %1, %2, %3" : "=v"(Cmb) : "v"(Ab), "s"(0x7F800000u), "v"(0x00400000u));
            const float Cm = __uint_as_float(Cmb);
            Bq2[e] = (t + Cm) - Cm;
          }
          const v2f x2 = {xq[i][j], xq[i][j + 1]};
          const v2f o2 = __builtin_elementwise_fma(T2, x2, Bq2);
          if (PM1) {
            q[j] = o2[0];
            q[j + 1] = o2[1];
          } else {
            q[j] = rintf(o2[0]) * p4[j];
            q[j + 1] = rintf(o2[1]) * p4[j + 1];
          }
          if constexpr (TAP) {
            ot[j] = rintf(o2[0]);
            ot[j + 1] = rintf(o2[1]);
          }
        }
        outw[i] = pack4_rne_sat(q[0], q[1], q[2], q[3]);
        if constexpr (TAP)
          if (tap && L.on[i]) ln_tap_store(tap, (l32 + LANES * i) * 4, ln, ot);
      }
    };
    if (L.pm_one) chain(std::integral_constant<bool, true>{});
    else chain(std::integral_constant<bool, false>{});
  } else {
#pragma unroll
    for (int i = 0; i < NCH; ++i) {
      const int cc = L.on[i] ? (l32 + LANES * i) * 4 : 0;
      const float4 gv = *reinterpret_cast<const float4*>(ln.gamma + cc), bv = *reinterpret_cast<const float4*>(ln.beta + cc);
      const float4 iv = *reinterpret_cast<const float4*>(ln.inv_out + cc), pv = *reinterpret_cast<const float4*>(ln.post_mul + cc);
      const float g4[4] = {gv.x, gv.y, gv.z, gv.w}, b4[4] = {bv.x, bv.y, bv.z, bv.w};
      const float i4[4] = {iv.x, iv.y, iv.z, iv.w}, p4[4] = {pv.x, pv.y, pv.z, pv.w};
      float4 ov = make_float4(0.f, 0.f, 0.f, 0.f);
      if (ln.out_scale) ov = *reinterpret_cast<const float4*>(ln.out_scale + cc);
      const float o4[4] = {ov.x, ov.y, ov.z, ov.w};
      float q[4];
      if constexpr (TAP) {
        float ot[4];
#pragma unroll
        for (int j = 0; j < 4; ++j) {
          ot[j] = ln_elem_generic_o(xq[i][j] * LN_XS_INV, g4[j], b4[j], i4[j], rs, mos, o4[j]);
          q[j] = rintf(ot[j] * p4[j]);
        }
        if (tap && L.on[i]) ln_tap_store(tap, cc, ln, ot);
      } else {
#pragma unroll
        for (int j = 0; j < 4; ++j) q[j] = ln_elem_generic(xq[i][j] * LN_XS_INV, g4[j], b4[j], i4[j], p4[j], rs, mos, o4[j]);
      }
      outw[i] = pack4_sat(q[0], q[1], q[2], q[3]);
    }
  }
}

template <int NCH, int LANES, class LL, bool TAP = false>
__device__ __forceinline__ void ln_row(const unsigned (&wcur)[NCH], const LL& L, const p2v_ln& ln, int C, int l32, unsigned (&outw)[NCH],
                                       float* tap = nullptr) {
  float xq[NCH][4], rs, mos;
  int S1;
  unsigned S2;
  bool fast;
  ln_sums<NCH>(wcur, L, xq, S1, S2);
  ln_reduce<LANES>(S1, S2);
  ln_scalars<NCH>(S1, S2, L, ln, C, rs, mos, fast);
  ln_apply<NCH, LANES, LL, TAP>(xq, L, ln, l32, rs, mos, fast, outw, tap);
}

template <int NCH, int LANES, int R, class LL, bool TAP = false>
__device__ __forceinline__ void ln_rows(const unsigned (&wcur)[R][NCH], const LL& L, const p2v_ln& ln, int C, int l32, unsigned (&outw)[R][NCH],
                                        float* const* taps = nullptr) {
  static_assert((R & (R - 1)) == 0 && R <= 8, "rows per batch");
  float xq[R][NCH][4];
  int S1k = 0;
  unsigned S2k = 0;
  const int mine = l32 & (R - 1);
#pragma unroll
  for (int r = 0; r < R; ++r) {
    int S1;
    unsigned S2;
    ln_sums<NCH>(wcur[r], L, xq[r], S1, S2);
    ln_reduce<LANES>(S1, S2);
    S1k = mine == r ? S1 : S1k;
    S2k = mine == r ? S2 : S2k;
  }
  float rs, mos;
  bool fast;
  ln_scalars<NCH>(S1k, S2k, L, ln, C, rs, mos, fast);
  const int fasti = fast ? 1 : 0;
#pragma unroll
  for (int r = 0; r < R; ++r) {
    const float rs_r = __shfl(rs, r, LANES), mos_r = __shfl(mos, r, LANES);
    const bool fast_r = __shfl(fasti, r, LANES) != 0;
    ln_apply<NCH, LANES, LL, TAP>(xq[r], L, ln, l32, rs_r, mos_r, fast_r, outw[r], TAP ? taps[r] : nullptr);
  }
}
```

Before: 107,700 images/sec.

## Add lean LN-GEMM kernel variants with paired DPP reductions behind a switch

Moves the fused layernorm+GEMM kernels into a shared header and adds lean kernel forms (VER 4/5) built in a separate translation unit, chosen through a new ln_gemm_lean switch. It also adds a half-wave reduction that sums two row statistics at once with DPP halving, cutting cross-lane shuffle instructions in the LN prologue. The goal is a shorter LN stage inside the fused kernel. The new code is large, and part of it is not visible here, so dispatch and correctness are hard to confirm.

```diff
diff --git a/diff-vit_amd/csrc/p2vit_capi.cpp b/diff-vit_amd/csrc/p2vit_capi.cpp
--- a/diff-vit_amd/csrc/p2vit_capi.cpp
+++ b/diff-vit_amd/csrc/p2vit_capi.cpp
@@ -139,6 +139,7 @@
 extern int g_attn_waves;
 extern int g_ln_gemm;
 extern int g_ln_gemm_ver;
+extern int g_ln_gemm_lean;
 extern int g_gemm_tile;
 extern int g_resid_pre;
 extern int g_attn_stream;
@@ -167,6 +168,7 @@
     {"cls_rows", "P2V_CLS_ROWS", &g_cls_rows, 0, 1, 1, ANY_ENV},
     {"ln_rows", "P2V_LN_ROWS", &g_ln_rows, 1, 64, 1, 0},
     {"ln_generic", "P2V_LN_GENERIC", &g_ln_generic, 0, 1, 1, ANY_API},
+    {"ln_gemm_lean", "P2V_LN_GEMM_LEAN", &g_ln_gemm_lean, 0, 1, 1, ANY_ENV | ANY_API},
 };
 
 static void read_env_once() {
diff --git a/diff-vit_amd/csrc/p2vit_ln.hip b/diff-vit_amd/csrc/p2vit_ln.hip
--- a/diff-vit_amd/csrc/p2vit_ln.hip
+++ b/diff-vit_amd/csrc/p2vit_ln.hip
@@ -111,480 +111,8 @@
   }
 }
 
-#define LG_BM 64
-template <bool W4> struct LgW { typedef uint4 raw; };
-template <> struct LgW<true> { typedef uint2 raw; };
-__device__ __forceinline__ v4i lg_wfrag(uint4 w) { return __builtin_bit_cast(v4i, w); }
-__device__ __forceinline__ v4i lg_wfrag(uint2 w) { return unpack_w4(w.x, w.y); }
-struct LnGemmLds {
-  int panel, consts, fold, table, total;
-};
-__host__ __device__ inline LnGemmLds ln_gemm_lds(int K, int N, int nch, int table_cells) {
-  LnGemmLds o;
-  const int kt = (K + GBK - 1) / GBK, tiles_n = (N + GBN - 1) / GBN;
-  o.panel = 0;
-  o.consts = o.panel + kt * LG_BM * GBK;
-  o.fold = o.panel;
-  o.table = o.consts + tiles_n * GBN * 2 * (int)sizeof(float);
-  o.total = o.table + table_cells * 8;
-  return o;
-}
+#include "p2vit_ln_gemm.h"
 
-#ifdef P2V_DIAG
-#define LG_STAMP(slot)                                                                                              \
-  do {                                                                                                              \
-    if (g.stamps && threadIdx.x == 0 && (slot) < 62) g.stamps[(long long)blockIdx.x * 64 + (slot)] = __builtin_readcyclecounter(); \
-  } while (0)
-#else
-#define LG_STAMP(slot) do { } while (0)
-#endif
-template <int EPI, int KT, bool W4>
-__global__ __launch_bounds__(256, 2) void k_ln_gemm(LnArgs a, GemmArgs g) {
-  typedef typename LgW<W4>::raw wraw;
-  constexpr int NCH = (KT + 1) / 2;
-  constexpr int NI = 2 * KT;
-  extern __shared__ __attribute__((aligned(1024))) unsigned char lg_smem[];
-  LG_STAMP(0);
-  const int C = a.C;
-  const int cells = EPI == P2V_EPI_GELU_TAB ? g.ep.gelu.cells : 0;
-  const LnGemmLds lay = ln_gemm_lds(C, g.N, NCH, cells);
-  int8_t* panel = reinterpret_cast<int8_t*>(lg_smem + lay.panel);
-  float* consts = reinterpret_cast<float*>(lg_smem + lay.consts);
-  const unsigned char* gtab = lg_smem + lay.table;
-  const int tid = threadIdx.x, lane = tid & 63;
-  const int wave = __builtin_amdgcn_readfirstlane(tid >> 6);
-  const int h = lane >> 5, l31 = lane & 31;
-  const int m0 = blockIdx.x * LG_BM;
-  const int tiles_n = g.tiles_n;
-
-  const wraw* wsrc = reinterpret_cast<const wraw*>(g.W) + (long long)wave * NI * 64 + lane;
-  wraw wf[NI];
-#pragma unroll
-  for (int i = 0; i < NI; ++i) wf[i] = wsrc[i * 64];
-
-  constexpr int RPH = LG_BM / 8;
-  static_assert(RPH % 2 == 0, "rows are processed in pairs");
-  const int hw = tid >> 5;
-  auto load_row = [&](int r, unsigned (&w)[NCH]) {
-    long long row = (long long)m0 + hw * RPH + r;
-    row = row < a.rows ? row : a.rows - 1;
-#pragma unroll
-    for (int i = 0; i < NCH; ++i) {
-      const int c = (l31 + 32 * i) * 4;
-      w[i] = *reinterpret_cast<const unsigned*>(a.x + row * a.row_stride + (c < C ? c : 0));
-    }
-  };
-  unsigned win[2][NCH];
-  load_row(0, win[0]);
-  load_row(1, win[1]);
-  {
-    const float fold = EPI == P2V_EPI_REQUANT ? g.ep.inv_s_out : (EPI == P2V_EPI_GELU_TAB ? g.ep.gelu.k : 1.0f);
-    const float cfold = fold * (W4 ? 0.0625f : 1.0f);
-    for (int n4 = tid; n4 < tiles_n * (GBN / 4); n4 += 256) {
-      const int j_ = n4 >> 5, c_ = (n4 & 31) * 4;
-      const float4 cv = *reinterpret_cast<const float4*>(g.colscale + n4 * 4);
-      const float4 bv = *reinterpret_cast<const float4*>(g.bias + n4 * 4);
-      *reinterpret_cast<float4*>(consts + j_ * 2 * GBN + c_) = make_float4(cv.x * cfold, cv.y * cfold, cv.z * cfold, cv.w * cfold);
-      *reinterpret_cast<float4*>(consts + j_ * 2 * GBN + GBN + c_) = make_float4(bv.x * fold, bv.y * fold, bv.z * fold, bv.w * fold);
-    }
-    if (EPI == P2V_EPI_GELU_TAB)
-      for (int i = tid; i < cells; i += 256)
-        reinterpret_cast<uint2*>(lg_smem + lay.table)[i] = reinterpret_cast<const uint2*>(g.ep.gelu.table)[i];
-  }
-  LG_STAMP(1);
-  {
-    float* sG = reinterpret_cast<float*>(lg_smem + lay.fold);
-    float* sB = sG + NCH * 128;
-    float* sP = sB + NCH * 128;
-    int* sM = reinterpret_cast<int*>(sP + NCH * 128);
-    LnLane<NCH> L;
-    ln_prepare<NCH, 32>(a.ln, C, a.force_generic != 0, sG, sB, sP, sM, tid, 256, L);
-    __syncthreads();
-#pragma unroll 1
-    for (int r = 0; r < RPH; r += 2) {
-      unsigned wnext[2][NCH];
-      if (r + 2 < RPH) {
-        load_row(r + 2, wnext[0]);
-        load_row(r + 3, wnext[1]);
-      }
-      unsigned wcur[2][NCH], outw2[2][NCH];
-#pragma unroll
-      for (int u = 0; u < 2; ++u)
-#pragma unroll
-        for (int i = 0; i < NCH; ++i) wcur[u][i] = L.on[i] ? win[u][i] : 0u;
-      ln_rows<NCH, 32, 2>(wcur, L, a.ln, C, l31, outw2);
-#pragma unroll
-      for (int u = 0; u < 2; ++u) {
-        const int lrow = hw * RPH + r + u;
-        const unsigned (&outw)[NCH] = outw2[u];
-        const long long row = (long long)m0 + lrow;
-#pragma unroll
-        for (int i = 0; i < NCH; ++i) {
-          const int c = (l31 + 32 * i) * 4;
-          if (c < KT * GBK)
-            *reinterpret_cast<unsigned*>(panel + (c >> 6) * (LG_BM * GBK) + lrow * GBK + ((((c & 63) >> 4) ^ ((lrow >> 2) & 3)) << 4) + (c & 15)) =
-                L.on[i] ? outw[i] : 0u;
-          if (a.out && L.on[i] && row < a.rows) *reinterpret_cast<unsigned*>(a.out + row * a.out_stride + c) = outw[i];
-        }
-      }
-      if (r + 2 < RPH) {
-#pragma unroll
-        for (int i = 0; i < NCH; ++i) {
-          win[0][i] = wnext[0][i];
-          win[1][i] = wnext[1][i];
-        }
-      }
-    }
-  }
-  LG_STAMP(2);
-  __syncthreads();
-  LG_STAMP(3);
-
-  const int8_t* pXa = panel + lds_off64(l31, h);
-  const int8_t* pXb = panel + lds_off64(32 + l31, h);
-  const int xks = (lds_off64(l31, 2 + h) - lds_off64(l31, h));
-  v16i acc[2];
-#pragma unroll
-  for (int b = 0; b < 2; ++b)
-#pragma unroll
-    for (int r = 0; r < 16; ++r) acc[b][r] = 0;
-
-  for (int j = 0; j < tiles_n; ++j) {
-    const bool more = j + 1 < tiles_n;
-    const wraw* wnext = wsrc + (long long)(more ? j + 1 : j) * 4 * NI * 64;
-#pragma unroll
-    for (int i = 0; i < NI; ++i) {
-      const int off = (i >> 1) * (LG_BM * GBK) + (i & 1) * xks;
-      const v4i xa = *reinterpret_cast<const v4i*>(pXa + off);
-      const v4i xb = *reinterpret_cast<const v4i*>(pXb + off);
-      const v4i wfi = lg_wfrag(wf[i]);
-      acc[0] = __builtin_amdgcn_mfma_i32_32x32x32_i8(wfi, xa, acc[0], 0, 0, 0);
-      acc[1] = __builtin_amdgcn_mfma_i32_32x32x32_i8(wfi, xb, acc[1], 0, 0, 0);
-      wf[i] = wnext[i * 64];
-    }
-    LG_STAMP(4 + 2 * j);
-    const EpiLds* e = reinterpret_cast<const EpiLds*>(consts + j * 2 * GBN);
-    {
-      const uint4 nores[2] = {make_uint4(0, 0, 0, 0), make_uint4(0, 0, 0, 0)};
-      gemm_epilogue_tile2<EPI>(acc, m0 + l31, j * GBN + 32 * wave, 32 * wave, h, g, e, nores, gtab);
-#pragma unroll
-      for (int mi = 0; mi < 2; ++mi)
-#pragma unroll
-        for (int r = 0; r < 16; ++r) acc[mi][r] = 0;
-    }
-    LG_STAMP(5 + 2 * j);
-  }
-}
-
-template <int NI>
-__host__ __device__ constexpr int lg2_mfma_at(int hp) {
-  for (int q = 0; q < 2 * NI; ++q)
-    if ((q * 12) / NI == hp) return q;
-  return -1;
-}
-
-#ifndef LG2_LN_ROWS
-#define LG2_LN_ROWS 2
-#endif
-template <int EPI, int KT, int NG, bool W4>
-__global__ __launch_bounds__(256 * NG, 2) void k_ln_gemm2(LnArgs a, GemmArgs g) {
-  typedef typename LgW<W4>::raw wraw;
-  constexpr int NT = 256 * NG;
-  static_assert(EPI == P2V_EPI_REQUANT || EPI == P2V_EPI_GELU_TAB, "pipelined epilogues");
-  constexpr int NCH = (KT + 1) / 2;
-  constexpr int NI = 2 * KT;
-  extern __shared__ __attribute__((aligned(1024))) unsigned char lg_smem[];
-  LG_STAMP(0);
-  const int C = a.C;
-  const int cells = EPI == P2V_EPI_GELU_TAB ? g.ep.gelu.cells : 0;
-  const LnGemmLds lay = ln_gemm_lds(C, g.N, NCH, cells);
-  int8_t* panel = reinterpret_cast<int8_t*>(lg_smem + lay.panel);
-  float* consts = reinterpret_cast<float*>(lg_smem + lay.consts);
-  const unsigned char* gtab = lg_smem + lay.table;
-  const int tid = threadIdx.x, lane = tid & 63;
-  const int wave = __builtin_amdgcn_readfirstlane(tid >> 6);
-  const int grp = NG == 1 ? 0 : (wave >> 2), cw = wave & 3;
-  const int h = lane >> 5, l31 = lane & 31;
-  const int m0 = blockIdx.x * LG_BM;
-  const int tiles_n = g.tiles_n;
-  const int n_g = (tiles_n - grp + NG - 1) / NG;
-
-  const wraw* wsrc = reinterpret_cast<const wraw*>(g.W) + (long long)cw * NI * 64 + lane;
-  auto wtile = [&](int it) {
-    int j = grp + NG * it;
-    j = j < tiles_n ? j : tiles_n - 1;
-    return wsrc + (long long)j * 4 * NI * 64;
-  };
-  constexpr int NI_EARLY = KT >= 6 ? NI - 1 : NI;
-  wraw wf[NI];
-  {
-    const wraw* w0 = wtile(0);
-#pragma unroll
-    for (int i = 0; i < NI_EARLY; ++i) wf[i] = w0[i * 64];
-  }
-
-  constexpr int RPH = LG_BM / (8 * NG);
-  static_assert(RPH % 2 == 0, "rows are processed in pairs");
-  const int hw = tid >> 5;
-  const int8_t* xblk = a.x + (long long)m0 * a.row_stride;
-  const int rstride = (int)a.row_stride;
-  const int last_lr = (int)(a.rows - 1 - m0);
-  auto load_row = [&](int r, unsigned (&w)[NCH]) {
-    int lr = hw * RPH + r;
-    lr = lr < last_lr ? lr : last_lr;
-    const int8_t* rp = xblk + lr * rstride;
-#pragma unroll
-    for (int i = 0; i < NCH; ++i) {
-      const int c = (l31 + 32 * i) * 4;
-      w[i] = *reinterpret_cast<const unsigned*>(rp + (c < C ? c : 0));
-    }
-  };
-  constexpr int LR = LG2_LN_ROWS < RPH ? LG2_LN_ROWS : RPH;
-  static_assert(RPH % LR == 0, "rows are processed in batches");
-  unsigned win[LR][NCH];
-#pragma unroll
-  for (int u = 0; u < LR; ++u) load_row(u, win[u]);
-  {
-    const float fold = EPI == P2V_EPI_REQUANT ? g.ep.inv_s_out : (EPI == P2V_EPI_GELU_TAB ? g.ep.gelu.k : 1.0f);
-    const float cfold = fold * (W4 ? 0.0625f : 1.0f);
-    for (int n4 = tid; n4 < tiles_n * (GBN / 4); n4 += NT) {
-      const int j_ = n4 >> 5, c_ = (n4 & 31) * 4;
-      const float4 cv = *reinterpret_cast<const float4*>(g.colscale + n4 * 4);
-      const float4 bv = *reinterpret_cast<const float4*>(g.bias + n4 * 4);
-      *reinterpret_cast<float4*>(consts + j_ * 2 * GBN + c_) = make_float4(cv.x * cfold, cv.y * cfold, cv.z * cfold, cv.w * cfold);
-      *reinterpret_cast<float4*>(consts + j_ * 2 * GBN + GBN + c_) = make_float4(bv.x * fold, bv.y * fold, bv.z * fold, bv.w * fold);
-    }
-    if (EPI == P2V_EPI_GELU_TAB)
-      for (int i = tid; i < cells; i += NT)
-        reinterpret_cast<uint2*>(lg_smem + lay.table)[i] = reinterpret_cast<const uint2*>(g.ep.gelu.table)[i];
-  }
-  LG_STAMP(1);
-  {
-    float* sG = reinterpret_cast<float*>(lg_smem + lay.fold);
-    float* sB = sG + NCH * 128;
-    float* sP = sB + NCH * 128;
-    int* sM = reinterpret_cast<int*>(sP + NCH * 128);
-    LnLane<NCH> L;
-    if (a.pre.gm) {
-#pragma unroll
-      for (int i = 0; i < NCH; ++i) {
-        const int c = (l31 + 32 * i) * 4;
-        L.on[i] = c < C;
-        L.gm[i] = *reinterpret_cast<const float4*>(a.pre.gm + c);
-        L.bt[i] = *reinterpret_cast<const float4*>(a.pre.bt + c);
-        L.pm[i] = L.on[i] ? *reinterpret_cast<const float4*>(a.ln.post_mul + c) : make_float4(0.f, 0.f, 0.f, 0.f);
-        L.mkf[i] = L.on[i] ? ln_scale_mask(*reinterpret_cast<const float4*>(a.ln.mask + c)) : make_float4(0.f, 0.f, 0.f, 0.f);
-      }
-      L.gmin = a.pre.gmin;
-      L.gmax = a.pre.gmax;
-      L.bmax = a.pre.bmax;
-      L.pot = a.pre.pot != 0 && a.force_generic == 0;
-      L.pm_one = a.pre.pm_one != 0;
-    } else {
-      ln_prepare<NCH, 32>(a.ln, C, a.force_generic != 0, sG, sB, sP, sM, tid, NT, L);
-      __syncthreads();
-    }
-#pragma unroll 1
-    for (int r = 0; r < RPH; r += LR) {
-      unsigned wnext[LR][NCH];
-      if (r + LR < RPH) {
-#pragma unroll
-        for (int u = 0; u < LR; ++u) load_row(r + LR + u, wnext[u]);
-      }
-      unsigned wcur[LR][NCH], outw2[LR][NCH];
-#pragma unroll
-      for (int u = 0; u < LR; ++u)
-#pragma unroll
-        for (int i = 0; i < NCH; ++i) wcur[u][i] = L.on[i] ? win[u][i] : 0u;
-      ln_rows<NCH, 32, LR>(wcur, L, a.ln, C, l31, outw2);
-#pragma unroll
-      for (int u = 0; u < LR; ++u) {
-        const int lrow = hw * RPH + r + u;
-        const unsigned (&outw)[NCH] = outw2[u];
-        const long long row = (long long)m0 + lrow;
-#pragma unroll
-        for (int i = 0; i < NCH; ++i) {
-          const int c = (l31 + 32 * i) * 4;
-          if (c < KT * GBK)
-            *reinterpret_cast<unsigned*>(panel + (c >> 6) * (LG_BM * GBK) + lrow * GBK + ((((c & 63) >> 4) ^ ((lrow >> 2) & 3)) << 4) + (c & 15)) =
-                L.on[i] ? outw[i] : 0u;
-          if (a.out && L.on[i] && row < a.rows) *reinterpret_cast<unsigned*>(a.out + row * a.out_stride + c) = outw[i];
-        }
-      }
-      if (r + LR < RPH) {
-#pragma unroll
-        for (int u = 0; u < LR; ++u)
-#pragma unroll
-          for (int i = 0; i < NCH; ++i) win[u][i] = wnext[u][i];
-      }
-    }
-  }
-  LG_STAMP(2);
-  if constexpr (NI_EARLY < NI) wf[NI - 1] = wtile(0)[(NI - 1) * 64];
-  __syncthreads();
-  LG_STAMP(3);
-  if (n_g <= 0) return;
-
-  const int8_t* pXa = panel + lds_off64(l31, h);
-  const int8_t* pXb = panel + lds_off64(32 + l31, h);
-  const int xks = (lds_off64(l31, 2 + h) - lds_off64(l31, h));
-#define LG2_XOFF(i) ((((i) >> 1) * (LG_BM * GBK)) + (((i) & 1) ? xks : 0))
-  v16i acc[2], accn[2];
-#pragma unroll
-  for (int b = 0; b < 2; ++b)
-#pragma unroll
-    for (int r = 0; r < 16; ++r) acc[b][r] = 0;
-  {
-    const wraw* wn = wtile(1);
-#pragma unroll
-    for (int i = 0; i < NI; ++i) {
-      const v4i xa = *reinterpret_cast<const v4i*>(pXa + LG2_XOFF(i));
-      const v4i xb = *reinterpret_cast<const v4i*>(pXb + LG2_XOFF(i));
-      const v4i wfi = lg_wfrag(wf[i]);
-      acc[0] = __builtin_amdgcn_mfma_i32_32x32x32_i8(wfi, xa, acc[0], 0, 0, 0);
-      acc[1] = __builtin_amdgcn_mfma_i32_32x32x32_i8(wfi, xb, acc[1], 0, 0, 0);
-      wf[i] = wn[i * 64];
-    }
-  }
-  LG_STAMP(4);
-  v4i XA[2], XB[2];
-  XA[0] = *reinterpret_cast<const v4i*>(pXa + LG2_XOFF(0));
-  XB[0] = *reinterpret_cast<const v4i*>(pXb + LG2_XOFF(0));
-  XA[1] = XA[0];
-  XB[1] = XB[0];
-  const int goff = (int)g.ep.gelu.off;
-  const float glo = (float)-goff, ghi = (float)(cells - 1 - goff) + 0.5f;
-  const unsigned char* gtabz = gtab + goff * 8;
-
-  v4i wcur = {0, 0, 0, 0};
-  auto tile_body = [&](auto MFc, auto LDc, auto COPYc, int j, const wraw* wnn, v16i (&acc)[2], v16i (&accn)[2]) {
-    constexpr bool MF = decltype(MFc)::value, LD = decltype(LDc)::value, COPY = decltype(COPYc)::value;
-    const float* cst = consts + j * 2 * GBN + 32 * cw + 4 * h;
-    const int n_tile = j * GBN + 32 * cw;
-    unsigned d[2][4];
-    float4 cs = *reinterpret_cast<const float4*>(cst), bs = *reinterpret_cast<const float4*>(cst + GBN);
-#define LG2_MFMA(HP)                                                                                                     \
-    do {                                                                                                                 \
-      constexpr int q_ = lg2_mfma_at<NI>(HP);                                                                            \
-      if constexpr (MF && q_ >= 0) {                                                                                     \
-        constexpr int i_ = q_ >> 1, nx_ = (i_ + 1) % NI;                                                                 \
-        if constexpr ((q_ & 1) == 0) {                                                                                   \
-          XA[nx_ & 1] = *reinterpret_cast<const v4i*>(pXa + LG2_XOFF(nx_));                                              \
-          wcur = lg_wfrag(wf[i_]);                                                                                       \
-          if constexpr (i_ == 0) accn[0] = __builtin_amdgcn_mfma_i32_32x32x32_i8(wcur, XA[i_ & 1], (v16i){0,0,0,0,0,0,0,0,0,0,0,0,0,0,0,0}, 0, 0, 0); \
-          else accn[0] = __builtin_amdgcn_mfma_i32_32x32x32_i8(wcur, XA[i_ & 1], accn[0], 0, 0, 0);                      \
-        } else {                                                                                                         \
-          XB[nx_ & 1] = *reinterpret_cast<const v4i*>(pXb + LG2_XOFF(nx_));                                              \
-          if constexpr (i_ == 0) accn[1] = __builtin_amdgcn_mfma_i32_32x32x32_i8(wcur, XB[i_ & 1], (v16i){0,0,0,0,0,0,0,0,0,0,0,0,0,0,0,0}, 0, 0, 0); \
-          else accn[1] = __builtin_amdgcn_mfma_i32_32x32x32_i8(wcur, XB[i_ & 1], accn[1], 0, 0, 0);                      \
-          if constexpr (LD) wf[i_] = wnn[i_ * 64];                                                                       \
-        }                                                                                                                \
-      }                                                                                                                  \
-    } while (0)
-#define LG2_FENCE() __builtin_amdgcn_sched_barrier(0)
-    auto group = [&](auto GQc) {
-      constexpr int gq = decltype(GQc)::value;
-      const float4 csc = cs, bsc = bs;
-      if (gq < 3) {
-        cs = *reinterpret_cast<const float4*>(cst + 8 * (gq + 1));
-        bs = *reinterpret_cast<const float4*>(cst + GBN + 8 * (gq + 1));
-      }
-      float y0[4], y1[4];
-      LG2_MFMA(6 * gq + 0);
-      y0[0] = __builtin_fmaf((float)acc[0][4 * gq + 0], csc.x, bsc.x);
-      y0[1] = __builtin_fmaf((float)acc[0][4 * gq + 1], csc.y, bsc.y);
-      y0[2] = __builtin_fmaf((float)acc[0][4 * gq + 2], csc.z, bsc.z);
-      y0[3] = __builtin_fmaf((float)acc[0][4 * gq + 3], csc.w, bsc.w);
-      LG2_FENCE();
-      LG2_MFMA(6 * gq + 1);
-      y1[0] = __builtin_fmaf((float)acc[1][4 * gq + 0], csc.x, bsc.x);
-      y1[1] = __builtin_fmaf((float)acc[1][4 * gq + 1], csc.y, bsc.y);
-      y1[2] = __builtin_fmaf((float)acc[1][4 * gq + 2], csc.z, bsc.z);
-      y1[3] = __builtin_fmaf((float)acc[1][4 * gq + 3], csc.w, bsc.w);
-      LG2_FENCE();
-      if constexpr (EPI == P2V_EPI_GELU_TAB) {
-        uint2 e0[4], e1[4];
-        LG2_MFMA(6 * gq + 2);
-#pragma unroll
-        for (int i = 0; i < 4; ++i) e0[i] = *reinterpret_cast<const uint2*>(gtabz + gelu_tab_offset(y0[i], glo, ghi));
-        LG2_FENCE();
-        LG2_MFMA(6 * gq + 3);
-#pragma unroll
-        for (int i = 0; i < 4; ++i) e1[i] = *reinterpret_cast<const uint2*>(gtabz + gelu_tab_offset(y1[i], glo, ghi));
-        LG2_FENCE();
-        LG2_MFMA(6 * gq + 4);
-        d[0][gq] = 0;
-        P2V_GELU_SEL(0, "UNUSED_PAD", d[0][gq], y0[0], e0[0]);
-        P2V_GELU_SEL(1, "UNUSED_PRESERVE", d[0][gq], y0[1], e0[1]);
-        P2V_GELU_SEL(2, "UNUSED_PRESERVE", d[0][gq], y0[2], e0[2]);
-        P2V_GELU_SEL(3, "UNUSED_PRESERVE", d[0][gq], y0[3], e0[3]);
-        LG2_FENCE();
-        LG2_MFMA(6 * gq + 5);
-        d[1][gq] = 0;
-        P2V_GELU_SEL(0, "UNUSED_PAD", d[1][gq], y1[0], e1[0]);
-        P2V_GELU_SEL(1, "UNUSED_PRESERVE", d[1][gq], y1[1], e1[1]);
-        P2V_GELU_SEL(2, "UNUSED_PRESERVE", d[1][gq], y1[2], e1[2]);
-        P2V_GELU_SEL(3, "UNUSED_PRESERVE", d[1][gq], y1[3], e1[3]);
-        LG2_FENCE();
-      } else {
-        float r0[4], r1[4];
-        LG2_MFMA(6 * gq + 2);
-#pragma unroll
-        for (int i = 0; i < 4; ++i) r0[i] = pre_pack(y0[i]);
-        LG2_FENCE();
-        LG2_MFMA(6 * gq + 3);
-#pragma unroll
-        for (int i = 0; i < 4; ++i) r1[i] = pre_pack(y1[i]);
-        LG2_FENCE();
-        LG2_MFMA(6 * gq + 4);
-        d[0][gq] = pack4_pre(r0[0], r0[1], r0[2], r0[3]);
-        LG2_FENCE();
-        LG2_MFMA(6 * gq + 5);
-        d[1][gq] = pack4_pre(r1[0], r1[1], r1[2], r1[3]);
-        LG2_FENCE();
-      }
-    };
-    group(std::integral_constant<int, 0>{});
-    group(std::integral_constant<int, 1>{});
-    group(std::integral_constant<int, 2>{});
-    group(std::integral_constant<int, 3>{});
-#undef LG2_MFMA
-#undef LG2_FENCE
-#pragma unroll
-    for (int b = 0; b < 2; ++b) {
-      const uint4 o = halves_to_row16(d[b][0], d[b][1], d[b][2], d[b][3]);
-      const int m = m0 + 32 * b + l31;
-      if (m < g.M && n_tile + 16 * h < g.N)
-        *reinterpret_cast<uint4*>(reinterpret_cast<int8_t*>(g.out) + (long long)m * g.ldo + n_tile + 16 * h) = o;
-    }
-    if constexpr (MF && COPY) {
-      acc[0] = accn[0];
-      acc[1] = accn[1];
-    }
-  };
-  using T_ = std::integral_constant<bool, true>;
-  using F_ = std::integral_constant<bool, false>;
-  int it = 0;
-  for (; it + 3 < n_g; it += 2) {
-    tile_body(T_{}, T_{}, F_{}, grp + NG * it, wtile(it + 2), acc, accn);
-    LG_STAMP(5 + it);
-    tile_body(T_{}, T_{}, F_{}, grp + NG * (it + 1), wtile(it + 3), accn, acc);
-    LG_STAMP(6 + it);
-  }
-  if (it + 2 < n_g) {
-    tile_body(T_{}, T_{}, T_{}, grp + NG * it, wtile(it + 2), acc, accn);
-    LG_STAMP(5 + it);
-    ++it;
-  }
-  if (it + 1 < n_g) {
-    tile_body(T_{}, F_{}, T_{}, grp + NG * it, wsrc, acc, accn);
-    LG_STAMP(5 + it);
-    ++it;
-  }
-  tile_body(F_{}, F_{}, T_{}, grp + NG * it, wsrc, acc, accn);
-  LG_STAMP(5 + it);
-#undef LG2_XOFF
-}
 
 
 #ifdef P2V_DIAG
@@ -598,23 +126,6 @@
   if (C % 4 || C > 384 || N % 16) return false;
   return ln_gemm_lds(C, N, ((C + GBK - 1) / GBK + 1) / 2, table_cells).total <= 80 * 1024;
 }
-template <int EPI, int KT, int VER, bool W4>
-static int launch_ln_gemm_t(const LnArgs& a, const GemmArgs& g, int cells, hipStream_t st) {
-  constexpr auto kernel = [] {
-    if constexpr (VER == 1) return &k_ln_gemm<EPI, KT, W4>;
-    else return &k_ln_gemm2<EPI, KT, VER - 1, W4>;
-  }();
-  const int smem = ln_gemm_lds(a.C, g.N, (KT + 1) / 2, cells).total;
-  static P2vLdsGrant grant = {};
-  const hipError_t e = grant.ensure(reinterpret_cast<const void*>(kernel), smem);
-  if (e != hipSuccess) return (int)e;
-  const dim3 grid((unsigned)((g.M + LG_BM - 1) / LG_BM));
-  hipLaunchKernelGGL(kernel, grid, dim3(VER == 3 ? 512 : 256), (unsigned)smem, st, a, g);
-  CHECK_LAUNCH();
-  return 0;
-}
-typedef int (*LnGemmLauncher)(const LnArgs&, const GemmArgs&, int, hipStream_t);
-constexpr int kLnGemmEpi[3] = {P2V_EPI_REQUANT, P2V_EPI_GELU_TAB, P2V_EPI_GELU};
 constexpr int ln_gemm_index(int e, int ver, int kt, bool w4) { return (((3 - ver) * 3 + p2v_slot(kLnGemmEpi, e)) * 6 + kt - 1) * 2 + (w4 ? 0 : 1); }
 struct LnGemmAt {
   template <int I> static constexpr LnGemmLauncher at() {
@@ -625,7 +136,7 @@
   }
 };
 static const auto ln_gemm_table = p2v_table<LnGemmLauncher, LnGemmAt, 108>();
-
+int g_ln_gemm_lean = 1;
 int g_ln_gemm_ver = 2;
 int p2v_launch_ln_gemm(int epi, const LnArgs& a_, const GemmArgs& g0, hipStream_t st) {
   const int cells = (epi == P2V_EPI_GELU && g0.ep.gelu.table) ? g0.ep.gelu.cells : 0;
@@ -642,7 +153,9 @@
   const int kt = (a.C + GBK - 1) / GBK;
   const int e = epi == P2V_EPI_REQUANT ? P2V_EPI_REQUANT : (cells ? P2V_EPI_GELU_TAB : P2V_EPI_GELU);
   const int ver = ((g_ln_gemm_ver == 3 || g_ln_gemm_ver == 2) && !g.ep.tap_out && e != P2V_EPI_GELU) ? g_ln_gemm_ver : 1;
-  const LnGemmLauncher launch = ln_gemm_table[ln_gemm_index(e, ver, kt >= 1 && kt <= 5 ? kt : 6, g.w4 != 0)];
+  const int kti = kt >= 1 && kt <= 5 ? kt : 6;
+  const bool lean = g_ln_gemm_lean && ver == 2 && a.pre.gm && a.pre.pot && !a.force_generic && a.C == kt * GBK && !a.out && !a.tap_out;
+  const LnGemmLauncher launch = lean ? p2v_ln_gemm_lean_launcher(e, a.pre.pm_one != 0, kti, g.w4 != 0) : ln_gemm_table[ln_gemm_index(e, ver, kti, g.w4 != 0)];
   return launch ? launch(a, g, cells, st) : -3;
 }
 
diff --git a/diff-vit_amd/csrc/p2vit_ln_gemm.h b/diff-vit_amd/csrc/p2vit_ln_gemm.h
--- /dev/null
+++ b/diff-vit_amd/csrc/p2vit_ln_gemm.h
@@ -0,0 +1,588 @@
+#pragma once
+#include "p2vit_ln_row.h"
+#include "p2vit_launch.h"
+
+#define LG_BM 64
+template <bool W4> struct LgW { typedef uint4 raw; };
+template <> struct LgW<true> { typedef uint2 raw; };
+__device__ __forceinline__ v4i lg_wfrag(uint4 w) { return __builtin_bit_cast(v4i, w); }
+__device__ __forceinline__ v4i lg_wfrag(uint2 w) { return unpack_w4(w.x, w.y); }
+struct LnGemmLds {
+  int panel, consts, fold, table, total;
+};
+__host__ __device__ inline LnGemmLds ln_gemm_lds(int K, int N, int nch, int table_cells) {
+  LnGemmLds o;
+  const int kt = (K + GBK - 1) / GBK, tiles_n = (N + GBN - 1) / GBN;
+  o.panel = 0;
+  o.consts = o.panel + kt * LG_BM * GBK;
+  o.fold = o.panel;
+  o.table = o.consts + tiles_n * GBN * 2 * (int)sizeof(float);
+  o.total = o.table + table_cells * 8;
+  return o;
+}
+
+#ifdef P2V_DIAG
+#define LG_STAMP(slot)                                                                                              \
+  do {                                                                                                              \
+    if (g.stamps && threadIdx.x == 0 && (slot) < 62) g.stamps[(long long)blockIdx.x * 64 + (slot)] = __builtin_readcyclecounter(); \
+  } while (0)
+#else
+#define LG_STAMP(slot) do { } while (0)
+#endif
+template <int EPI, int KT, bool W4>
+__global__ __launch_bounds__(256, 2) void k_ln_gemm(LnArgs a, GemmArgs g) {
+  typedef typename LgW<W4>::raw wraw;
+  constexpr int NCH = (KT + 1) / 2;
+  constexpr int NI = 2 * KT;
+  extern __shared__ __attribute__((aligned(1024))) unsigned char lg_smem[];
+  LG_STAMP(0);
+  const int C = a.C;
+  const int cells = EPI == P2V_EPI_GELU_TAB ? g.ep.gelu.cells : 0;
+  const LnGemmLds lay = ln_gemm_lds(C, g.N, NCH, cells);
+  int8_t* panel = reinterpret_cast<int8_t*>(lg_smem + lay.panel);
+  float* consts = reinterpret_cast<float*>(lg_smem + lay.consts);
+  const unsigned char* gtab = lg_smem + lay.table;
+  const int tid = threadIdx.x, lane = tid & 63;
+  const int wave = __builtin_amdgcn_readfirstlane(tid >> 6);
+  const int h = lane >> 5, l31 = lane & 31;
+  const int m0 = blockIdx.x * LG_BM;
+  const int tiles_n = g.tiles_n;
+
+  const wraw* wsrc = reinterpret_cast<const wraw*>(g.W) + (long long)wave * NI * 64 + lane;
+  wraw wf[NI];
+#pragma unroll
+  for (int i = 0; i < NI; ++i) wf[i] = wsrc[i * 64];
+
+  constexpr int RPH = LG_BM / 8;
+  static_assert(RPH % 2 == 0, "rows are processed in pairs");
+  const int hw = tid >> 5;
+  auto load_row = [&](int r, unsigned (&w)[NCH]) {
+    long long row = (long long)m0 + hw * RPH + r;
+    row = row < a.rows ? row : a.rows - 1;
+#pragma unroll
+    for (int i = 0; i < NCH; ++i) {
+      const int c = (l31 + 32 * i) * 4;
+      w[i] = *reinterpret_cast<const unsigned*>(a.x + row * a.row_stride + (c < C ? c : 0));
+    }
+  };
+  unsigned win[2][NCH];
+  load_row(0, win[0]);
+  load_row(1, win[1]);
+  {
+    const float fold = EPI == P2V_EPI_REQUANT ? g.ep.inv_s_out : (EPI == P2V_EPI_GELU_TAB ? g.ep.gelu.k : 1.0f);
+    const float cfold = fold * (W4 ? 0.0625f : 1.0f);
+    for (int n4 = tid; n4 < tiles_n * (GBN / 4); n4 += 256) {
+      const int j_ = n4 >> 5, c_ = (n4 & 31) * 4;
+      const float4 cv = *reinterpret_cast<const float4*>(g.colscale + n4 * 4);
+      const float4 bv = *reinterpret_cast<const float4*>(g.bias + n4 * 4);
+      *reinterpret_cast<float4*>(consts + j_ * 2 * GBN + c_) = make_float4(cv.x * cfold, cv.y * cfold, cv.z * cfold, cv.w * cfold);
+      *reinterpret_cast<float4*>(consts + j_ * 2 * GBN + GBN + c_) = make_float4(bv.x * fold, bv.y * fold, bv.z * fold, bv.w * fold);
+    }
+    if (EPI == P2V_EPI_GELU_TAB)
+      for (int i = tid; i < cells; i += 256)
+        reinterpret_cast<uint2*>(lg_smem + lay.table)[i] = reinterpret_cast<const uint2*>(g.ep.gelu.table)[i];
+  }
+  LG_STAMP(1);
+  {
+    float* sG = reinterpret_cast<float*>(lg_smem + lay.fold);
+    float* sB = sG + NCH * 128;
+    float* sP = sB + NCH * 128;
+    int* sM = reinterpret_cast<int*>(sP + NCH * 128);
+    LnLane<NCH> L;
+    ln_prepare<NCH, 32>(a.ln, C, a.force_generic != 0, sG, sB, sP, sM, tid, 256, L);
+    __syncthreads();
+#pragma unroll 1
+    for (int r = 0; r < RPH; r += 2) {
+      unsigned wnext[2][NCH];
+      if (r + 2 < RPH) {
+        load_row(r + 2, wnext[0]);
+        load_row(r + 3, wnext[1]);
+      }
+      unsigned wcur[2][NCH], outw2[2][NCH];
+#pragma unroll
+      for (int u = 0; u < 2; ++u)
+#pragma unroll
+        for (int i = 0; i < NCH; ++i) wcur[u][i] = L.on[i] ? win[u][i] : 0u;
+      ln_rows<NCH, 32, 2>(wcur, L, a.ln, C, l31, outw2);
+#pragma unroll
+      for (int u = 0; u < 2; ++u) {
+        const int lrow = hw * RPH + r + u;
+        const unsigned (&outw)[NCH] = outw2[u];
+        const long long row = (long long)m0 + lrow;
+#pragma unroll
+        for (int i = 0; i < NCH; ++i) {
+          const int c = (l31 + 32 * i) * 4;
+          if (c < KT * GBK)
+            *reinterpret_cast<unsigned*>(panel + (c >> 6) * (LG_BM * GBK) + lrow * GBK + ((((c & 63) >> 4) ^ ((lrow >> 2) & 3)) << 4) + (c & 15)) =
+                L.on[i] ? outw[i] : 0u;
+          if (a.out && L.on[i] && row < a.rows) *reinterpret_cast<unsigned*>(a.out + row * a.out_stride + c) = outw[i];
+        }
+      }
+      if (r + 2 < RPH) {
+#pragma unroll
+        for (int i = 0; i < NCH; ++i) {
+          win[0][i] = wnext[0][i];
+          win[1][i] = wnext[1][i];
+        }
+      }
+    }
+  }
+  LG_STAMP(2);
+  __syncthreads();
+  LG_STAMP(3);
+
+  const int8_t* pXa = panel + lds_off64(l31, h);
+  const int8_t* pXb = panel + lds_off64(32 + l31, h);
+  const int xks = (lds_off64(l31, 2 + h) - lds_off64(l31, h));
+  v16i acc[2];
+#pragma unroll
+  for (int b = 0; b < 2; ++b)
+#pragma unroll
+    for (int r = 0; r < 16; ++r) acc[b][r] = 0;
+
+  for (int j = 0; j < tiles_n; ++j) {
+    const bool more = j + 1 < tiles_n;
+    const wraw* wnext = wsrc + (long long)(more ? j + 1 : j) * 4 * NI * 64;
+#pragma unroll
+    for (int i = 0; i < NI; ++i) {
+      const int off = (i >> 1) * (LG_BM * GBK) + (i & 1) * xks;
+      const v4i xa = *reinterpret_cast<const v4i*>(pXa + off);
+      const v4i xb = *reinterpret_cast<const v4i*>(pXb + off);
+      const v4i wfi = lg_wfrag(wf[i]);
+      acc[0] = __builtin_amdgcn_mfma_i32_32x32x32_i8(wfi, xa, acc[0], 0, 0, 0);
+      acc[1] = __builtin_amdgcn_mfma_i32_32x32x32_i8(wfi, xb, acc[1], 0, 0, 0);
+      wf[i] = wnext[i * 64];
+    }
+    LG_STAMP(4 + 2 * j);
+    const EpiLds* e = reinterpret_cast<const EpiLds*>(consts + j * 2 * GBN);
+    {
+      const uint4 nores[2] = {make_uint4(0, 0, 0, 0), make_uint4(0, 0, 0, 0)};
+      gemm_epilogue_tile2<EPI>(acc, m0 + l31, j * GBN + 32 * wave, 32 * wave, h, g, e, nores, gtab);
+#pragma unroll
+      for (int mi = 0; mi < 2; ++mi)
+#pragma unroll
+        for (int r = 0; r < 16; ++r) acc[mi][r] = 0;
+    }
+    LG_STAMP(5 + 2 * j);
+  }
+}
+
+template <int NI>
+__host__ __device__ constexpr int lg2_mfma_at(int hp) {
+  for (int q = 0; q < 2 * NI; ++q)
+    if ((q * 12) / NI == hp) return q;
+  return -1;
+}
+
+#ifndef LG2_LN_ROWS
+#define LG2_LN_ROWS 2
+#endif
+#define LG2_FORM_LEAN 3
+#define LG2_FORM_LEAN_PM1 4
+template <int EPI, int KT, int FORM, bool W4>
+__global__ __launch_bounds__(256 * (FORM == 2 ? 2 : 1), 2) void k_ln_gemm2(LnArgs a, GemmArgs g) {
+  typedef typename LgW<W4>::raw wraw;
+  constexpr int NG = FORM == 2 ? 2 : 1;
+  constexpr bool LEAN = FORM >= LG2_FORM_LEAN, PM1 = FORM == LG2_FORM_LEAN_PM1;
+  constexpr int NT = 256 * NG;
+  static_assert(EPI == P2V_EPI_REQUANT || EPI == P2V_EPI_GELU_TAB, "pipelined epilogues");
+  static_assert(FORM >= 1 && FORM <= LG2_FORM_LEAN_PM1, "forms");
+  constexpr int NCH = (KT + 1) / 2;
+  constexpr int NI = 2 * KT;
+  extern __shared__ __attribute__((aligned(1024))) unsigned char lg_smem[];
+  LG_STAMP(0);
+  const int C = LEAN ? KT * GBK : a.C;
+  const int cells = EPI == P2V_EPI_GELU_TAB ? g.ep.gelu.cells : 0;
+  const LnGemmLds lay = ln_gemm_lds(C, g.N, NCH, cells);
+  int8_t* panel = reinterpret_cast<int8_t*>(lg_smem + lay.panel);
+  float* consts = reinterpret_cast<float*>(lg_smem + lay.consts);
+  const unsigned char* gtab = lg_smem + lay.table;
+  const int tid = threadIdx.x, lane = tid & 63;
+  const int wave = __builtin_amdgcn_readfirstlane(tid >> 6);
+  const int grp = NG == 1 ? 0 : (wave >> 2), cw = wave & 3;
+  const int h = lane >> 5, l31 = lane & 31;
+  const int m0 = blockIdx.x * LG_BM;
+  const int tiles_n = g.tiles_n;
+  const int n_g = (tiles_n - grp + NG - 1) / NG;
+
+  const wraw* wsrc = reinterpret_cast<const wraw*>(g.W) + (long long)cw * NI * 64 + lane;
+  auto wtile = [&](int it) {
+    int j = grp + NG * it;
+    j = j < tiles_n ? j : tiles_n - 1;
+    return wsrc + (long long)j * 4 * NI * 64;
+  };
+  constexpr int NI_EARLY = KT >= 6 ? NI - 1 : NI;
+  wraw wf[NI];
+  {
+    const wraw* w0 = wtile(0);
+#pragma unroll
+    for (int i = 0; i < NI_EARLY; ++i) wf[i] = w0[i * 64];
+  }
+
+  constexpr int RPH = LG_BM / (8 * NG);
+  static_assert(RPH % 2 == 0, "rows are processed in pairs");
+  const int hw = tid >> 5;
+  const int8_t* xblk = a.x + (long long)m0 * a.row_stride;
+  const int rstride = (int)a.row_stride;
+  const int last_lr = (int)(a.rows - 1 - m0);
+  auto load_row = [&](int r, unsigned (&w)[NCH]) {
+    int lr = hw * RPH + r;
+    lr = lr < last_lr ? lr : last_lr;
+    const int8_t* rp = xblk + lr * rstride;
+#pragma unroll
+    for (int i = 0; i < NCH; ++i) {
+      const int c = (l31 + 32 * i) * 4;
+      w[i] = *reinterpret_cast<const unsigned*>(rp + (c < C ? c : 0));
+    }
+  };
+  constexpr int LR = LG2_LN_ROWS < RPH ? LG2_LN_ROWS : RPH;
+  static_assert(RPH % LR == 0, "rows are processed in batches");
+  unsigned win[LR][NCH];
+  constexpr bool ODD_LAST = (KT & 1) != 0;
+  [[maybe_unused]] unsigned wnx[LR][NCH];
+  [[maybe_unused]] const bool lane_last_on = !ODD_LAST || l31 < 16;
+  [[maybe_unused]] const unsigned row0_off = (unsigned)(hw * RPH * rstride + l31 * 4);
+  [[maybe_unused]] const unsigned last_off = (unsigned)((last_lr < LG_BM - 1 ? last_lr : LG_BM - 1) * rstride + l31 * 4);
+  [[maybe_unused]] const unsigned last_col = lane_last_on ? (unsigned)(128 * (NCH - 1)) : (unsigned)(-l31 * 4);
+  auto lean_load = [&](int r, unsigned (&w)[LR][NCH]) {
+#pragma unroll
+    for (int u = 0; u < LR; ++u) {
+      unsigned ro = row0_off + (unsigned)((r + u) * rstride);
+      ro = ro < last_off ? ro : last_off;
+#pragma unroll
+      for (int i = 0; i < NCH; ++i) {
+        if (ODD_LAST && i == NCH - 1) w[u][i] = *reinterpret_cast<const unsigned*>(xblk + (ro + last_col));
+        else w[u][i] = *reinterpret_cast<const unsigned*>(xblk + 128 * i + ro);
+      }
+    }
+  };
+  if constexpr (LEAN) {
+    lean_load(0, win);
+  } else {
+#pragma unroll
+    for (int u = 0; u < LR; ++u) load_row(u, win[u]);
+  }
+  {
+    const float fold = EPI == P2V_EPI_REQUANT ? g.ep.inv_s_out : (EPI == P2V_EPI_GELU_TAB ? g.ep.gelu.k : 1.0f);
+    const float cfold = fold * (W4 ? 0.0625f : 1.0f);
+    for (int n4 = tid; n4 < tiles_n * (GBN / 4); n4 += NT) {
+      const int j_ = n4 >> 5, c_ = (n4 & 31) * 4;
+      const float4 cv = *reinterpret_cast<const float4*>(g.colscale + n4 * 4);
+      const float4 bv = *reinterpret_cast<const float4*>(g.bias + n4 * 4);
+      *reinterpret_cast<float4*>(consts + j_ * 2 * GBN + c_) = make_float4(cv.x * cfold, cv.y * cfold, cv.z * cfold, cv.w * cfold);
+      *reinterpret_cast<float4*>(consts + j_ * 2 * GBN + GBN + c_) = make_float4(bv.x * fold, bv.y * fold, bv.z * fold, bv.w * fold);
+    }
+    if (EPI == P2V_EPI_GELU_TAB)
+      for (int i = tid; i < cells; i += NT)
+        reinterpret_cast<uint2*>(lg_smem + lay.table)[i] = reinterpret_cast<const uint2*>(g.ep.gelu.table)[i];
+  }
+  LG_STAMP(1);
+  if constexpr (LEAN) {
+    static_assert(RPH == 8 && LR == 2, "two turns of two row pairs; the panel swizzle below");
+    LnLane<NCH> L;
+#pragma unroll
+    for (int i = 0; i < NCH; ++i) {
+      const int c = (l31 + 32 * i) * 4;
+      L.on[i] = (ODD_LAST && i == NCH - 1) ? lane_last_on : true;
+      L.gm[i] = *reinterpret_cast<const float4*>(a.pre.gm + c);
+      L.bt[i] = *reinterpret_cast<const float4*>(a.pre.bt + c);
+      if constexpr (!PM1) L.pm[i] = L.on[i] ? *reinterpret_cast<const float4*>(a.ln.post_mul + c) : make_float4(0.f, 0.f, 0.f, 0.f);
+      L.mkf[i] = L.on[i] ? ln_scale_mask(*reinterpret_cast<const float4*>(a.ln.mask + c)) : make_float4(0.f, 0.f, 0.f, 0.f);
+    }
+    L.gmin = a.pre.gmin;
+    L.gmax = a.pre.gmax;
+    L.bmax = a.pre.bmax;
+    L.pot = true;
+    L.pm_one = PM1;
+    const int pbase = (l31 >> 4) * (LG_BM * GBK) + hw * RPH * GBK + (l31 & 3) * 4;
+    const int pofs[2] = {pbase + ((((l31 >> 2) & 3) ^ ((2 * hw) & 3)) << 4), pbase + 4 * GBK + ((((l31 >> 2) & 3) ^ ((2 * hw + 1) & 3)) << 4)};
+    const int src_lane[2] = {(tid & 32) * 4, ((tid & 32) + 8) * 4};
+    auto pair = [&](int turn, auto Rc, unsigned (&cur)[LR][NCH], unsigned (&nxt)[LR][NCH]) {
+      constexpr int r = decltype(Rc)::value;
+      if (r == 0 || turn == 0) lean_load(4 * turn + r + 2, nxt);
+      float xq[2][NCH][4];
+      int S1[2], S1k;
+      unsigned S2[2], S2k;
+      ln_sums<NCH>(cur[0], L, xq[0], S1[0], S2[0]);
+      ln_sums<NCH>(cur[1], L, xq[1], S1[1], S2[1]);
+      half_wave_sum_pair(S1, S2, S1k, S2k);
+      float rs, mos;
+      bool fast;
+      ln_scalars<NCH>(S1k, S2k, L, a.ln, C, rs, mos, fast);
+      float rs_u[2], mos_u[2];
+#pragma unroll
+      for (int u = 0; u < 2; ++u) {
+        rs_u[u] = __int_as_float(__builtin_amdgcn_ds_bpermute(src_lane[u], __float_as_int(rs)));
+        mos_u[u] = __int_as_float(__builtin_amdgcn_ds_bpermute(src_lane[u], __float_as_int(mos)));
+      }
+      unsigned outw[2][NCH];
+      if (__builtin_expect((__builtin_amdgcn_ballot_w64(!fast) & 0x0F0F0F0F0F0F0F0Full) != 0, 0)) {
+        const int fasti = fast ? 1 : 0;
+#pragma unroll
+        for (int u = 0; u < 2; ++u) {
+          const bool fast_u = __builtin_amdgcn_ds_bpermute(src_lane[u], fasti) != 0;
+          ln_apply<NCH, 32>(xq[u], L, a.ln, l31, rs_u[u], mos_u[u], fast_u, outw[u]);
+        }
+      } else {
+#pragma unroll
+        for (int u = 0; u < 2; ++u) ln_apply<NCH, 32>(xq[u], L, a.ln, l31, rs_u[u], mos_u[u], true, outw[u]);
+      }
+      int8_t* prow = panel + (turn ? pofs[1] : pofs[0]);
+#pragma unroll
+      for (int u = 0; u < 2; ++u)
+#pragma unroll
+        for (int i = 0; i < NCH; ++i)
+          if (!(ODD_LAST && i == NCH - 1) || lane_last_on)
+            *reinterpret_cast<unsigned*>(prow + (r + u) * GBK + 2 * i * (LG_BM * GBK)) = outw[u][i];
+    };
+#pragma unroll 1
+    for (int turn = 0; turn < 2; ++turn) {
+      pair(turn, std::integral_constant<int, 0>{}, win, wnx);
+      pair(turn, std::integral_constant<int, 2>{}, wnx, win);
+    }
+  } else {
+    float* sG = reinterpret_cast<float*>(lg_smem + lay.fold);
+    float* sB = sG + NCH * 128;
+    float* sP = sB + NCH * 128;
+    int* sM = reinterpret_cast<int*>(sP + NCH * 128);
+    LnLane<NCH> L;
+    if (a.pre.gm) {
+#pragma unroll
+      for (int i = 0; i < NCH; ++i) {
+        const int c = (l31 + 32 * i) * 4;
+        L.on[i] = c < C;
+        L.gm[i] = *reinterpret_cast<const float4*>(a.pre.gm + c);
+        L.bt[i] = *reinterpret_cast<const float4*>(a.pre.bt + c);
+        L.pm[i] = L.on[i] ? *reinterpret_cast<const float4*>(a.ln.post_mul + c) : make_float4(0.f, 0.f, 0.f, 0.f);
+        L.mkf[i] = L.on[i] ? ln_scale_mask(*reinterpret_cast<const float4*>(a.ln.mask + c)) : make_float4(0.f, 0.f, 0.f, 0.f);
+      }
+      L.gmin = a.pre.gmin;
+      L.gmax = a.pre.gmax;
+      L.bmax = a.pre.bmax;
+      L.pot = a.pre.pot != 0 && a.force_generic == 0;
+      L.pm_one = a.pre.pm_one != 0;
+    } else {
+      ln_prepare<NCH, 32>(a.ln, C, a.force_generic != 0, sG, sB, sP, sM, tid, NT, L);
+      __syncthreads();
+    }
+#pragma unroll 1
+    for (int r = 0; r < RPH; r += LR) {
+      unsigned wnext[LR][NCH];
+      if (r + LR < RPH) {
+#pragma unroll
+        for (int u = 0; u < LR; ++u) load_row(r + LR + u, wnext[u]);
+      }
+      unsigned wcur[LR][NCH], outw2[LR][NCH];
+#pragma unroll
+      for (int u = 0; u < LR; ++u)
+#pragma unroll
+        for (int i = 0; i < NCH; ++i) wcur[u][i] = L.on[i] ? win[u][i] : 0u;
+      ln_rows<NCH, 32, LR>(wcur, L, a.ln, C, l31, outw2);
+#pragma unroll
+      for (int u = 0; u < LR; ++u) {
+        const int lrow = hw * RPH + r + u;
+        const unsigned (&outw)[NCH] = outw2[u];
+        const long long row = (long long)m0 + lrow;
+#pragma unroll
+        for (int i = 0; i < NCH; ++i) {
+          const int c = (l31 + 32 * i) * 4;
+          if (c < KT * GBK)
+            *reinterpret_cast<unsigned*>(panel + (c >> 6) * (LG_BM * GBK) + lrow * GBK + ((((c & 63) >> 4) ^ ((lrow >> 2) & 3)) << 4) + (c & 15)) =
+                L.on[i] ? outw[i] : 0u;
+          if (a.out && L.on[i] && row < a.rows) *reinterpret_cast<unsigned*>(a.out + row * a.out_stride + c) = outw[i];
+        }
+      }
+      if (r + LR < RPH) {
+#pragma unroll
+        for (int u = 0; u < LR; ++u)
+#pragma unroll
+          for (int i = 0; i < NCH; ++i) win[u][i] = wnext[u][i];
+      }
+    }
+  }
+  LG_STAMP(2);
+  if constexpr (NI_EARLY < NI) wf[NI - 1] = wtile(0)[(NI - 1) * 64];
+  __syncthreads();
+  LG_STAMP(3);
+  if (n_g <= 0) return;
+
+  const int8_t* pXa = panel + lds_off64(l31, h);
+  const int8_t* pXb = panel + lds_off64(32 + l31, h);
+  const int xks = (lds_off64(l31, 2 + h) - lds_off64(l31, h));
+#define LG2_XOFF(i) ((((i) >> 1) * (LG_BM * GBK)) + (((i) & 1) ? xks : 0))
+  v16i acc[2], accn[2];
+#pragma unroll
+  for (int b = 0; b < 2; ++b)
+#pragma unroll
+    for (int r = 0; r < 16; ++r) acc[b][r] = 0;
+  {
+    const wraw* wn = wtile(1);
+#pragma unroll
+    for (int i = 0; i < NI; ++i) {
+      const v4i xa = *reinterpret_cast<const v4i*>(pXa + LG2_XOFF(i));
+      const v4i xb = *reinterpret_cast<const v4i*>(pXb + LG2_XOFF(i));
+      const v4i wfi = lg_wfrag(wf[i]);
+      acc[0] = __builtin_amdgcn_mfma_i32_32x32x32_i8(wfi, xa, acc[0], 0, 0, 0);
+      acc[1] = __builtin_amdgcn_mfma_i32_32x32x32_i8(wfi, xb, acc[1], 0, 0, 0);
+      wf[i] = wn[i * 64];
+    }
+  }
+  LG_STAMP(4);
+  v4i XA[2], XB[2];
+  XA[0] = *reinterpret_cast<const v4i*>(pXa + LG2_XOFF(0));
+  XB[0] = *reinterpret_cast<const v4i*>(pXb + LG2_XOFF(0));
+  XA[1] = XA[0];
+  XB[1] = XB[0];
+  const int goff = (int)g.ep.gelu.off;
+  const float glo = (float)-goff, ghi = (float)(cells - 1 - goff) + 0.5f;
+  const unsigned char* gtabz = gtab + goff * 8;
+
+  v4i wcur = {0, 0, 0, 0};
+  auto tile_body = [&](auto MFc, auto LDc, auto COPYc, int j, const wraw* wnn, v16i (&acc)[2], v16i (&accn)[2]) {
+    constexpr bool MF = decltype(MFc)::value, LD = decltype(LDc)::value, COPY = decltype(COPYc)::value;
+    const float* cst = consts + j * 2 * GBN + 32 * cw + 4 * h;
+    const int n_tile = j * GBN + 32 * cw;
+    unsigned d[2][4];
+    float4 cs = *reinterpret_cast<const float4*>(cst), bs = *reinterpret_cast<const float4*>(cst + GBN);
+#define LG2_MFMA(HP)                                                                                                     \
+    do {                                                                                                                 \
+      constexpr int q_ = lg2_mfma_at<NI>(HP);                                                                            \
+      if constexpr (MF && q_ >= 0) {                                                                                     \
+        constexpr int i_ = q_ >> 1, nx_ = (i_ + 1) % NI;                                                                 \
+        if constexpr ((q_ & 1) == 0) {                                                                                   \
+          XA[nx_ & 1] = *reinterpret_cast<const v4i*>(pXa + LG2_XOFF(nx_));                                              \
+          wcur = lg_wfrag(wf[i_]);                                                                                       \
+          if constexpr (i_ == 0) accn[0] = __builtin_amdgcn_mfma_i32_32x32x32_i8(wcur, XA[i_ & 1], (v16i){0,0,0,0,0,0,0,0,0,0,0,0,0,0,0,0}, 0, 0, 0); \
+          else accn[0] = __builtin_amdgcn_mfma_i32_32x32x32_i8(wcur, XA[i_ & 1], accn[0], 0, 0, 0);                      \
+        } else {                                                                                                         \
+          XB[nx_ & 1] = *reinterpret_cast<const v4i*>(pXb + LG2_XOFF(nx_));                                              \
+          if constexpr (i_ == 0) accn[1] = __builtin_amdgcn_mfma_i32_32x32x32_i8(wcur, XB[i_ & 1], (v16i){0,0,0,0,0,0,0,0,0,0,0,0,0,0,0,0}, 0, 0, 0); \
+          else accn[1] = __builtin_amdgcn_mfma_i32_32x32x32_i8(wcur, XB[i_ & 1], accn[1], 0, 0, 0);                      \
+          if constexpr (LD) wf[i_] = wnn[i_ * 64];                                                                       \
+        }                                                                                                                \
+      }                                                                                                                  \
+    } while (0)
+#define LG2_FENCE() __builtin_amdgcn_sched_barrier(0)
+    auto group = [&](auto GQc) {
+      constexpr int gq = decltype(GQc)::value;
+      const float4 csc = cs, bsc = bs;
+      if (gq < 3) {
+        cs = *reinterpret_cast<const float4*>(cst + 8 * (gq + 1));
+        bs = *reinterpret_cast<const float4*>(cst + GBN + 8 * (gq + 1));
+      }
+      float y0[4], y1[4];
+      LG2_MFMA(6 * gq + 0);
+      y0[0] = __builtin_fmaf((float)acc[0][4 * gq + 0], csc.x, bsc.x);
+      y0[1] = __builtin_fmaf((float)acc[0][4 * gq + 1], csc.y, bsc.y);
+      y0[2] = __builtin_fmaf((float)acc[0][4 * gq + 2], csc.z, bsc.z);
+      y0[3] = __builtin_fmaf((float)acc[0][4 * gq + 3], csc.w, bsc.w);
+      LG2_FENCE();
+      LG2_MFMA(6 * gq + 1);
+      y1[0] = __builtin_fmaf((float)acc[1][4 * gq + 0], csc.x, bsc.x);
+      y1[1] = __builtin_fmaf((float)acc[1][4 * gq + 1], csc.y, bsc.y);
+      y1[2] = __builtin_fmaf((float)acc[1][4 * gq + 2], csc.z, bsc.z);
+      y1[3] = __builtin_fmaf((float)acc[1][4 * gq + 3], csc.w, bsc.w);
+      LG2_FENCE();
+      if constexpr (EPI == P2V_EPI_GELU_TAB) {
+        uint2 e0[4], e1[4];
+        LG2_MFMA(6 * gq + 2);
+#pragma unroll
+        for (int i = 0; i < 4; ++i) e0[i] = *reinterpret_cast<const uint2*>(gtabz + gelu_tab_offset(y0[i], glo, ghi));
+        LG2_FENCE();
+        LG2_MFMA(6 * gq + 3);
+#pragma unroll
+        for (int i = 0; i < 4; ++i) e1[i] = *reinterpret_cast<const uint2*>(gtabz + gelu_tab_offset(y1[i], glo, ghi));
+        LG2_FENCE();
+        LG2_MFMA(6 * gq + 4);
+        d[0][gq] = 0;
+        P2V_GELU_SEL(0, "UNUSED_PAD", d[0][gq], y0[0], e0[0]);
+        P2V_GELU_SEL(1, "UNUSED_PRESERVE", d[0][gq], y0[1], e0[1]);
+        P2V_GELU_SEL(2, "UNUSED_PRESERVE", d[0][gq], y0[2], e0[2]);
+        P2V_GELU_SEL(3, "UNUSED_PRESERVE", d[0][gq], y0[3], e0[3]);
+        LG2_FENCE();
+        LG2_MFMA(6 * gq + 5);
+        d[1][gq] = 0;
+        P2V_GELU_SEL(0, "UNUSED_PAD", d[1][gq], y1[0], e1[0]);
+        P2V_GELU_SEL(1, "UNUSED_PRESERVE", d[1][gq], y1[1], e1[1]);
+        P2V_GELU_SEL(2, "UNUSED_PRESERVE", d[1][gq], y1[2], e1[2]);
+        P2V_GELU_SEL(3, "UNUSED_PRESERVE", d[1][gq], y1[3], e1[3]);
+        LG2_FENCE();
+      } else {
+        float r0[4], r1[4];
+        LG2_MFMA(6 * gq + 2);
+#pragma unroll
+        for (int i = 0; i < 4; ++i) r0[i] = pre_pack(y0[i]);
+        LG2_FENCE();
+        LG2_MFMA(6 * gq + 3);
+#pragma unroll
+        for (int i = 0; i < 4; ++i) r1[i] = pre_pack(y1[i]);
+        LG2_FENCE();
+        LG2_MFMA(6 * gq + 4);
+        d[0][gq] = pack4_pre(r0[0], r0[1], r0[2], r0[3]);
+        LG2_FENCE();
+        LG2_MFMA(6 * gq + 5);
+        d[1][gq] = pack4_pre(r1[0], r1[1], r1[2], r1[3]);
+        LG2_FENCE();
+      }
+    };
+    group(std::integral_constant<int, 0>{});
+    group(std::integral_constant<int, 1>{});
+    group(std::integral_constant<int, 2>{});
+    group(std::integral_constant<int, 3>{});
+#undef LG2_MFMA
+#undef LG2_FENCE
+#pragma unroll
+    for (int b = 0; b < 2; ++b) {
+      const uint4 o = halves_to_row16(d[b][0], d[b][1], d[b][2], d[b][3]);
+      const int m = m0 + 32 * b + l31;
+      if (m < g.M && n_tile + 16 * h < g.N)
+        *reinterpret_cast<uint4*>(reinterpret_cast<int8_t*>(g.out) + (long long)m * g.ldo + n_tile + 16 * h) = o;
+    }
+    if constexpr (MF && COPY) {
+      acc[0] = accn[0];
+      acc[1] = accn[1];
+    }
+  };
+  using T_ = std::integral_constant<bool, true>;
+  using F_ = std::integral_constant<bool, false>;
+  int it = 0;
+  for (; it + 3 < n_g; it += 2) {
+    tile_body(T_{}, T_{}, F_{}, grp + NG * it, wtile(it + 2), acc, accn);
+    LG_STAMP(5 + it);
+    tile_body(T_{}, T_{}, F_{}, grp + NG * (it + 1), wtile(it + 3), accn, acc);
+    LG_STAMP(6 + it);
+  }
+  if (it + 2 < n_g) {
+    tile_body(T_{}, T_{}, T_{}, grp + NG * it, wtile(it + 2), acc, accn);
+    LG_STAMP(5 + it);
+    ++it;
+  }
+  if (it + 1 < n_g) {
+    tile_body(T_{}, F_{}, T_{}, grp + NG * it, wsrc, acc, accn);
+    LG_STAMP(5 + it);
+    ++it;
+  }
+  tile_body(F_{}, F_{}, T_{}, grp + NG * it, wsrc, acc, accn);
+  LG_STAMP(5 + it);
+#undef LG2_XOFF
+}
+
+template <int EPI, int KT, int VER, bool W4>
+static int launch_ln_gemm_t(const LnArgs& a, const GemmArgs& g, int cells, hipStream_t st) {
+  static_assert(LG2_FORM_LEAN == 3 && LG2_FORM_LEAN_PM1 == 4, "VER - 1 is the form");
+  constexpr auto kernel = [] {
+    if constexpr (VER == 1) return &k_ln_gemm<EPI, KT, W4>;
+    else return &k_ln_gemm2<EPI, KT, VER - 1, W4>;
+  }();
+  const int smem = ln_gemm_lds(a.C, g.N, (KT + 1) / 2, cells).total;
+  static P2vLdsGrant grant = {};
+  const hipError_t e = grant.ensure(reinterpret_cast<const void*>(kernel), smem);
+  if (e != hipSuccess) return (int)e;
+  const dim3 grid((unsigned)((g.M + LG_BM - 1) / LG_BM));
+  hipLaunchKernelGGL(kernel, grid, dim3(VER == 3 ? 512 : 256), (unsigned)smem, st, a, g);
+  CHECK_LAUNCH();
+  return 0;
+}
+typedef int (*LnGemmLauncher)(const LnArgs&, const GemmArgs&, int, hipStream_t);
+constexpr int kLnGemmEpi[3] = {P2V_EPI_REQUANT, P2V_EPI_GELU_TAB, P2V_EPI_GELU};
+LnGemmLauncher p2v_ln_gemm_lean_launcher(int e, bool pm1, int kt, bool w4);
diff --git a/diff-vit_amd/csrc/p2vit_ln_lean.hip b/diff-vit_amd/csrc/p2vit_ln_lean.hip
--- /dev/null
+++ b/diff-vit_amd/csrc/p2vit_ln_lean.hip
@@ -0,0 +1,12 @@
+#include "p2vit_ln_gemm.h"
+
+constexpr int ln_gemm_lean_index(int e, bool pm1, int kt, bool w4) { return (((pm1 ? 0 : 1) * 2 + p2v_slot(kLnGemmEpi, e)) * 6 + kt - 1) * 2 + (w4 ? 0 : 1); }
+struct LnGemmLeanAt {
+  template <int I> static constexpr LnGemmLauncher at() {
+    constexpr int E = kLnGemmEpi[I / 12 % 2];
+    static_assert(ln_gemm_lean_index(E, I < 24, I / 2 % 6 + 1, !(I & 1)) == I, "decoded as the launcher encodes");
+    return launch_ln_gemm_t<E, I / 2 % 6 + 1, I < 24 ? 5 : 4, !(I & 1)>;
+  }
+};
+static const auto ln_gemm_lean_table = p2v_table<LnGemmLauncher, LnGemmLeanAt, 48>();
+LnGemmLauncher p2v_ln_gemm_lean_launcher(int e, bool pm1, int kt, bool w4) { return ln_gemm_lean_table[ln_gemm_lean_index(e, pm1, kt, w4)]; }
diff --git a/diff-vit_amd/csrc/p2vit_ln_row.h b/diff-vit_amd/csrc/p2vit_ln_row.h
--- a/diff-vit_amd/csrc/p2vit_ln_row.h
+++ b/diff-vit_amd/csrc/p2vit_ln_row.h
@@ -8,6 +8,23 @@
   v += __builtin_amdgcn_update_dpp(0, v, 0x140, 0xF, 0xF, false);
   v += __builtin_amdgcn_ds_swizzle(v, 0x401F);
   return v;
+}
+
+template <int CTRL, int BANKS_P>
+__device__ __forceinline__ int dpp_halve(int p, int q) {
+  const int x = __builtin_amdgcn_update_dpp(q, p, CTRL, 0xF, BANKS_P, false);
+  const int y = __builtin_amdgcn_update_dpp(p, q, CTRL, 0xF, BANKS_P ^ 0xF, false);
+  return x + y;
+}
+__device__ __forceinline__ void half_wave_sum_pair(const int (&S1)[2], const unsigned (&S2)[2], int& S1k, unsigned& S2k) {
+  const int a = dpp_halve<0x140, 0x3>(S1[0], S1[1]);
+  const int b = dpp_halve<0x140, 0x3>((int)S2[0], (int)S2[1]);
+  int v = dpp_halve<0x141, 0x5>(a, b);
+  v += __builtin_amdgcn_update_dpp(0, v, 0xB1, 0xF, 0xF, false);
+  v += __builtin_amdgcn_update_dpp(0, v, 0x4E, 0xF, 0xF, false);
+  v += __builtin_amdgcn_ds_swizzle(v, 0x401F);
+  S1k = v;
+  S2k = (unsigned)__builtin_amdgcn_update_dpp(0, v, 0x141, 0xF, 0xF, false);
 }
 
 __device__ __forceinline__ float ln_elem_generic_o(float xq, float g, float bta, float io, float rs, float mos, float os) {
```

New measurement: 108,800 images/sec (median of 6 runs). +1.1%, better.
